# Giuseppe5/brevitas

Measured on AMD Instinct MI355X. Metric: Gelem/s fused int8 fake-quant fwd+bwd, per-channel, [256,512,56,56], higher is better.
Workload: dtype bf16

## Files before the change

### brevitas_amd/_native.py

```python
import ctypes
import os

import torch

_PKG = os.path.dirname(os.path.abspath(__file__))
LIB_PATH = os.environ.get('BREVITAS_AMD_LIB') or os.path.join(_PKG, 'libbvq.so')

F32, BF16, F16 = 0, 1, 2
ROUND, FLOOR, CEIL, ROUND_TO_ZERO, DPU_ROUND = range(5)
(OP_ROUND, OP_FLOOR, OP_CEIL, OP_ROUND_TO_ZERO, OP_DPU_ROUND, OP_BINARY_SIGN, OP_TERNARY_SIGN,
 OP_ABS) = range(8)
STAT_ABSMAX, STAT_MINMAX = 0, 1
SCALAR_OPMATH, SCALAR_CAST = 0, 1
OUT_DEQUANT, OUT_INT = 0, 1
MATCH_ABS, MATCH_VALUE = 0, 1
MATCH_FIRST = 16
PRE_NONE, PRE_RELU = 0, 1
CODES_I32, CODES_I8, CODES_U8 = 0, 1, 2
_CODES_TORCH = {CODES_I32: torch.int32, CODES_I8: torch.int8, CODES_U8: torch.uint8}
ABI_VERSION = 2

_DTYPES = {torch.float32: F32, torch.bfloat16: BF16, torch.float16: F16}

EXPORTS = (
    'bvq_abi_version', 'bvq_last_error', 'bvq_unary', 'bvq_stats_pre', 'bvq_scalar_clamp', 'bvq_tensor_clamp',
    'bvq_tensor_clamp_bwd', 'bvq_abs_binary_sign_grad_bwd', 'bvq_stats_workspace_bytes', 'bvq_stats',
    'bvq_absmax_scale', 'bvq_running_stats_update', 'bvq_scale_from_stat', 'bvq_shard_pack', 'bvq_shard_unpack', 'bvq_abs_moments_workspace_bytes', 'bvq_abs_moments',
    'bvq_abs_affine_bwd', 'bvq_kth_workspace_bytes', 'bvq_kth_value', 'bvq_kth_pair', 'bvq_kth_passes',
    'bvq_kth_hist_offset', 'bvq_kth_begin', 'bvq_kth_hist', 'bvq_kth_pick', 'bvq_kth_finish', 'bvq_stat_bwd', 'bvq_tie_info_bytes', 'bvq_stat_tie_scan', 'bvq_stat_tie_apply', 'bvq_stat_tie_apply_dscale', 'bvq_fakequant_fwd', 'bvq_stats_fakequant_fwd_workspace_bytes', 'bvq_stats_fakequant_fwd',
    'bvq_fakequant_bwd_workspace_bytes', 'bvq_fakequant_bwd_stats_workspace_bytes', 'bvq_fakequant_bwd_stats', 'bvq_fakequant_bwd',
    'bvq_learned_scale', 'bvq_fakequant_bwd_learned', 'bvq_variant_fwd', 'bvq_variant_bwd_workspace_bytes', 'bvq_variant_bwd',
    'bvq_fakequant_fwd_bounds', 'bvq_fakequant_bwd_bounds', 'bvq_histc', 'bvq_absmax_scale_running', 'bvq_selftest_div_f16r',
    'bvq_kthw_plan', 'bvq_kthw_begin', 'bvq_kthw_hist', 'bvq_kthw_pick', 'bvq_kthw_finish',
    'bvq_absmax_onepass_supported', 'bvq_absmax_scale_onepass', 'bvq_fakequant_bwd_stats_onepass_supported',
    'bvq_fakequant_bwd_stats_onepass', 'bvq_scale_from_stat_running', 'bvq_fakequant_bwd_shard',
    'bvq_shard_unpack_deposit', 'bvq_absmax_list_supported', 'bvq_absmax_scale_list', 'bvq_weight_list_supported',
    'bvq_weight_quant_list_fwd', 'bvq_weight_quant_list_bwd_workspace_bytes', 'bvq_weight_quant_list_bwd')


class QuantDesc(ctypes.Structure):
    _fields_ = [
        ('outer', ctypes.c_int64), ('channels', ctypes.c_int64), ('inner', ctypes.c_int64),
        ('x_dtype', ctypes.c_int32), ('ct_dtype', ctypes.c_int32), ('scale_dtype', ctypes.c_int32),
        ('zp_dtype', ctypes.c_int32), ('scale_per_channel', ctypes.c_int32),
        ('zp_per_channel', ctypes.c_int32), ('qmin', ctypes.c_float), ('qmax', ctypes.c_float),
        ('round_mode', ctypes.c_int32), ('scalar_mode', ctypes.c_int32), ('clamp_ste', ctypes.c_int32),
        ('out_kind', ctypes.c_int32), ('pre_op', ctypes.c_int32), ('codes_dtype', ctypes.c_int32)]


class VariantDesc(ctypes.Structure):
    _fields_ = [
        ('outer', ctypes.c_int64), ('channels', ctypes.c_int64), ('inner', ctypes.c_int64), ('kind', ctypes.c_int32),
        ('x_dtype', ctypes.c_int32), ('ct_dtype', ctypes.c_int32), ('scale_dtype', ctypes.c_int32),
        ('zp_dtype', ctypes.c_int32), ('scale_per_channel', ctypes.c_int32), ('round_mode', ctypes.c_int32),
        ('clamp_ste', ctypes.c_int32), ('scalar_mode', ctypes.c_int32), ('qmin', ctypes.c_float),
        ('qmax', ctypes.c_float), ('threshold', ctypes.c_float), ('trunc_scale', ctypes.c_float)]


VAR_BINARY, VAR_CLAMPED_BINARY, VAR_TERNARY, VAR_DECOUPLED, VAR_TRUNC = range(5)

WEIGHT_LIST_MAX = 16


class WeightItem(ctypes.Structure):
    _fields_ = [
        ('x', ctypes.c_void_p), ('y', ctypes.c_void_p), ('stat', ctypes.c_void_p), ('scale', ctypes.c_void_p),
        ('g', ctypes.c_void_p), ('dx', ctypes.c_void_p), ('dscale', ctypes.c_void_p), ('channels', ctypes.c_int64),
        ('inner', ctypes.c_int64), ('min_val', ctypes.c_double), ('int_threshold', ctypes.c_double),
        ('qmin', ctypes.c_float), ('qmax', ctypes.c_float), ('use_min', ctypes.c_int32), ('clamp_ste', ctypes.c_int32)]


class BvqError(RuntimeError):
    pass


def _load(path=None, strict=True):
    path = path or LIB_PATH
    if not os.path.exists(path):
        raise ImportError(
            'brevitas_amd: %s is missing. Build it with `python -m brevitas_amd.csrc.build` '
            '(needs hipcc, gfx950). There is no fallback backend.' % path)
    lib = ctypes.CDLL(path)
    vp, i64, i32, dbl = ctypes.c_void_p, ctypes.c_int64, ctypes.c_int, ctypes.c_double
    lib.bvq_abi_version.restype = i32
    lib.bvq_last_error.restype = ctypes.c_char_p
    sig = {
        'bvq_unary': (i32, [i32, i32, vp, vp, i64, vp]),
        'bvq_scalar_clamp': (i32, [i32, vp, vp, i64, dbl, i32, dbl, i32, vp]),
        'bvq_tensor_clamp': (i32, [i32, vp, vp, vp, i32, vp, i64, vp]),
        'bvq_tensor_clamp_bwd': (i32, [i32, vp, vp, vp, vp, i32, vp, i64, vp]),
        'bvq_abs_binary_sign_grad_bwd': (i32, [i32, vp, vp, vp, i64, vp]),
        'bvq_stats_workspace_bytes': (i64, [i32, i32, i64, i64, i64]),
        'bvq_stats': (i32, [i32, i32, vp, i64, i64, i64, i32, vp, vp, i64, vp]),
        'bvq_stats_pre': (i32, [i32, i32, i32, vp, i64, i64, i64, i32, vp, vp, i64, vp]),
        'bvq_stat_bwd': (i32, [i32, i32, vp, vp, vp, vp, i64, i64, i64, i32, vp, i64, vp]),
        'bvq_fakequant_fwd': (i32, [ctypes.POINTER(QuantDesc), vp, vp, vp, vp, vp, vp]),
        'bvq_stats_fakequant_fwd_workspace_bytes': (i64, [ctypes.POINTER(QuantDesc), vp, vp]),
        'bvq_stats_fakequant_fwd': (i32, [ctypes.POINTER(QuantDesc), vp, dbl, i32, dbl, vp, vp, vp, vp, i64, vp]),
        'bvq_fakequant_bwd_workspace_bytes': (i64, [ctypes.POINTER(QuantDesc)]),
        'bvq_fakequant_bwd_stats_workspace_bytes': (i64, [ctypes.POINTER(QuantDesc)]),
        'bvq_fakequant_bwd_stats': (i32, [ctypes.POINTER(QuantDesc), vp, vp, vp, vp, vp, vp, vp, i32, dbl, i32, vp, i64, vp]),
        'bvq_fakequant_bwd_stats_onepass_supported': (i32, [ctypes.POINTER(QuantDesc)]),
        'bvq_fakequant_bwd_stats_onepass': (i32, [ctypes.POINTER(QuantDesc), vp, vp, vp, vp, vp, vp, vp, i32, dbl, i32, vp, i64, vp, i64, vp]),
        'bvq_absmax_scale': (i32, [i32, i32, vp, i64, i64, i64, vp, dbl, i32, dbl, i32, vp, vp, i64, vp]),
        'bvq_absmax_scale_running': (i32, [i32, i32, vp, i64, i64, i64, vp, dbl, i32, dbl, i32, vp, i32, vp, dbl, i32, vp, i64, vp]),
        'bvq_absmax_onepass_supported': (i32, [i32, vp, i64, i64, i64]),
        'bvq_absmax_scale_onepass': (i32, [i32, i32, vp, i64, i64, i64, i32, vp, dbl, i32, dbl, i32, vp, i32, vp, dbl, i32, vp, i64, vp]),
        'bvq_absmax_list_supported': (i32, [i32, i32, vp, vp, i64, vp]),
        'bvq_absmax_scale_list': (i32, [i32, i32, vp, vp, i64, vp, vp, dbl, i32, dbl, i32, vp, vp, i64, vp, i64, vp]),
        'bvq_running_stats_update': (i32, [i32, vp, i32, vp, i64, dbl, i32, vp]),
        'bvq_scale_from_stat': (i32, [vp, i64, i32, vp, dbl, i32, dbl, i32, vp, vp]),
        'bvq_scale_from_stat_running': (i32, [vp, i64, i32, vp, dbl, i32, dbl, i32, vp, i32, vp, dbl, i32, vp]),
        'bvq_fakequant_bwd_shard': (i32, [ctypes.POINTER(QuantDesc), vp, vp, vp, vp, vp, vp, vp, vp, i32, vp, i64, vp, i64, vp]),
        'bvq_shard_unpack_deposit': (i32, [i32, vp, vp, vp, i32, i64, i32, vp, i64, i32, dbl, i32, i32, vp, vp]),
        'bvq_shard_pack': (i32, [vp, vp, i64, i32, i32, vp, vp]),
        'bvq_shard_unpack': (i32, [vp, i32, i64, i32, i32, vp, vp, vp, vp]),
        'bvq_abs_moments_workspace_bytes': (i64, [i32, i64, i64, i64]),
        'bvq_abs_moments': (i32, [i32, vp, i64, i64, i64, vp, vp, i64, vp]),
        'bvq_abs_affine_bwd': (i32, [i32, vp, vp, vp, vp, i64, i64, i64, vp]),
        'bvq_kth_workspace_bytes': (i64, [i32, i64, i64, i64]),
        'bvq_kth_value': (i32, [i32, i32, vp, i64, i64, i64, i64, vp, vp, i64, vp]),
        'bvq_kth_pair': (i32, [i32, i32, vp, i64, i64, i64, i64, i64, vp, vp, i64, vp]),
        'bvq_kth_passes': (i32, [i32]),
        'bvq_kth_hist_offset': (i64, [i32, i64, i32]),
        'bvq_kth_begin': (i32, [i32, i64, i32, i64, dbl, vp, i64, vp]),
        'bvq_kth_hist': (i32, [i32, i32, vp, i64, i64, i64, i32, vp, i64, vp]),
        'bvq_kth_pick': (i32, [i32, i64, i32, i32, dbl, vp, i64, vp]),
        'bvq_kth_finish': (i32, [i32, i32, i64, vp, vp, i64, vp]),
        'bvq_kthw_plan': (i32, [i32, i32, i32, vp, vp]),
        'bvq_kthw_begin': (i32, [i32, i32, vp, i64, vp]),
        'bvq_kthw_hist': (i32, [i32, i32, vp, i64, i32, vp, i64, vp]),
        'bvq_kthw_pick': (i32, [i32, i32, i32, i32, i64, dbl, vp, i64, vp]),
        'bvq_kthw_finish': (i32, [i32, i32, vp, vp, i64, vp]),
        'bvq_tie_info_bytes': (i64, [i64]),
        'bvq_stat_tie_scan': (i32, [i32, i32, vp, vp, i64, i64, i64, vp, vp, vp]),
        'bvq_stat_tie_apply': (i32, [i32, i32, i32, vp, vp, vp, vp, vp, vp, i64, i64, i64, i32, vp]),
        'bvq_stat_tie_apply_dscale': (i32, [i32, i32, vp, vp, vp, i32, dbl, i32, vp, vp, vp, i64, i64, i64, vp]),
        'bvq_fakequant_bwd': (i32, [ctypes.POINTER(QuantDesc), vp, vp, vp, vp, vp, vp, vp, vp, vp, vp, i64, vp]),
        'bvq_learned_scale': (i32, [i32, vp, i64, dbl, i32, dbl, i32, vp, vp]),
        'bvq_histc': (i32, [i32, vp, i64, vp, i32, vp, vp]),
        'bvq_selftest_div_f16r': (i32, [vp, i32, vp, i32, vp, vp]),
        'bvq_fakequant_fwd_bounds': (i32, [ctypes.POINTER(QuantDesc), vp, vp, vp, vp, vp, vp]),
        'bvq_fakequant_bwd_bounds': (i32, [ctypes.POINTER(QuantDesc), vp, vp, vp, vp, vp, vp, vp, vp, vp, i64, vp]),
        'bvq_variant_fwd': (i32, [ctypes.POINTER(VariantDesc), vp, vp, vp, vp, vp, vp, vp]),
        'bvq_variant_bwd_workspace_bytes': (i64, [ctypes.POINTER(VariantDesc)]),
        'bvq_variant_bwd': (i32, [ctypes.POINTER(VariantDesc), vp, vp, vp, vp, vp, vp, vp, vp, vp, vp, i64, vp]),
        'bvq_weight_list_supported': (i32, [i32, i32, i32, vp, i64]),
        'bvq_weight_quant_list_fwd': (i32, [i32, i32, i32, i32, vp, vp]),
        'bvq_weight_quant_list_bwd_workspace_bytes': (i64, [i32, i32, vp]),
        'bvq_weight_quant_list_bwd': (i32, [i32, i32, i32, i32, i32, vp, vp, i64, vp, i64, vp]),
        'bvq_fakequant_bwd_learned': (i32, [ctypes.POINTER(QuantDesc), vp, vp, vp, vp, vp, vp, vp, i32, dbl, i32, dbl, vp, vp, vp, i64, vp]),
    }
    for name, (res, args) in sig.items():
        fn = getattr(lib, name, None)
        if fn is None:
            if strict:
                raise ImportError('brevitas_amd: %s does not export %s' % (path, name))
            continue
        fn.restype = res
        fn.argtypes = args
    ver = lib.bvq_abi_version()
    if ver != ABI_VERSION:
        raise ImportError('brevitas_amd: libbvq.so has ABI %d, this package needs %d' % (ver, ABI_VERSION))
    return lib


lib = _load()


def last_error():
    return lib.bvq_last_error().decode()


def check(rc, what):
    if rc != 0:
        raise BvqError('%s failed (%d): %s' % (what, rc, last_error()))


def dtype_code(dtype):
    try:
        return _DTYPES[dtype]
    except KeyError:
        raise BvqError('brevitas_amd: unsupported dtype %s (float32, bfloat16, float16)' % dtype)


def require_device(*tensors):
    dev = None
    for t in tensors:
        if t is None:
            continue
        if not t.is_cuda:
            raise BvqError(
                'brevitas_amd: got a %s tensor; the fake-quantization engine only runs on a ROCm '
                'device (there is no CPU fallback)' % t.device)
        if dev is None:
            dev = t.device
        elif t.device != dev:
            raise BvqError('brevitas_amd: tensors on different devices (%s, %s)' % (dev, t.device))
    return dev


_raw_stream = getattr(torch._C, '_cuda_getCurrentRawStream', None)


def stream_ptr(device):
    if _raw_stream is not None:
        return _raw_stream(device.index if device.index is not None else torch.cuda.current_device())
    return torch.cuda.current_stream(device).cuda_stream


def ptr(t):
    return t.data_ptr() if t is not None else None


class _DeviceGuard:
    __slots__ = ('ctx',)

    def __init__(self, dev):
        idx = dev.index
        self.ctx = None if idx is None or idx == torch.cuda.current_device() else torch.cuda.device(dev)

    def __enter__(self):
        if self.ctx is not None:
            self.ctx.__enter__()

    def __exit__(self, *exc):
        if self.ctx is not None:
            self.ctx.__exit__(*exc)
        return False


_timer = None


def set_kernel_timer(timer):
    global _timer
    _timer = timer


ARRIVE_WORDS = 1 << 16
_arrive = {}
ONEPASS = True
ONEPASS_BWD = True


def arrival_buffer(dev, stream, words):
    if not ONEPASS or words > ARRIVE_WORDS:
        return None
    key = (dev.index, stream)
    buf = _arrive.get(key)
    if buf is None:
        if torch.cuda.is_current_stream_capturing():
            return None
        buf = _arrive[key] = torch.zeros(ARRIVE_WORDS, dtype=torch.int32, device=dev)
    return buf



def unary(op, x):
    dev = require_device(x)
    x = x.contiguous()
    y = torch.empty_like(x)
    with _DeviceGuard(dev):
        check(lib.bvq_unary(op, dtype_code(x.dtype), ptr(x), ptr(y), x.numel(), stream_ptr(dev)), 'bvq_unary')
    return y


def scalar_clamp(x, lo, hi):
    dev = require_device(x)
    x = x.contiguous()
    y = torch.empty_like(x)
    with _DeviceGuard(dev):
        check(lib.bvq_scalar_clamp(dtype_code(x.dtype), ptr(x), ptr(y), x.numel(),
                                   0.0 if lo is None else float(lo), int(lo is not None),
                                   0.0 if hi is None else float(hi), int(hi is not None), stream_ptr(dev)),
              'bvq_scalar_clamp')
    return y


def _bounds(x, lo, hi):
    lo = lo.to(device=x.device, dtype=x.dtype)
    hi = hi.to(device=x.device, dtype=x.dtype)
    if lo.numel() == 1 and hi.numel() == 1:
        return lo.reshape(1), hi.reshape(1), 0
    return lo.expand_as(x).contiguous(), hi.expand_as(x).contiguous(), 1


def tensor_clamp(x, lo, hi, out=None):
    dev = require_device(x)
    xc = x.contiguous()
    lo, hi, full = _bounds(xc, lo, hi)
    y = out if out is not None else torch.empty_like(xc)
    with _DeviceGuard(dev):
        check(lib.bvq_tensor_clamp(dtype_code(xc.dtype), ptr(xc), ptr(lo), ptr(hi), full, ptr(y), xc.numel(),
                                   stream_ptr(dev)), 'bvq_tensor_clamp')
    return y


def tensor_clamp_bwd(g, x, lo, hi):
    dev = require_device(g, x)
    xc = x.contiguous()
    g = g.to(xc.dtype).contiguous()
    lo, hi, full = _bounds(xc, lo, hi)
    dx = torch.empty_like(xc)
    with _DeviceGuard(dev):
        check(lib.bvq_tensor_clamp_bwd(dtype_code(xc.dtype), ptr(g), ptr(xc), ptr(lo), ptr(hi), full, ptr(dx),
                                       xc.numel(), stream_ptr(dev)), 'bvq_tensor_clamp_bwd')
    return dx


def abs_binary_sign_grad_bwd(g, x):
    dev = require_device(g, x)
    xc = x.contiguous()
    g = g.to(xc.dtype).contiguous()
    dx = torch.empty_like(xc)
    with _DeviceGuard(dev):
        check(lib.bvq_abs_binary_sign_grad_bwd(dtype_code(xc.dtype), ptr(g), ptr(xc), ptr(dx), xc.numel(),
                                               stream_ptr(dev)), 'bvq_abs_binary_sign_grad_bwd')
    return dx


def stats(kind, x, outer, channels, inner, out_f32=False, pre_op=PRE_NONE):
    dev = require_device(x)
    assert x.is_contiguous() and x.numel() == outer * channels * inner
    dt = dtype_code(x.dtype)
    nout = channels * (2 if kind == STAT_MINMAX else 1)
    out = torch.empty(nout, dtype=torch.float32 if out_f32 else x.dtype, device=dev)
    if kind == STAT_ABSMAX and lib.bvq_absmax_onepass_supported(dt, ptr(x), outer, channels, inner):
        with _DeviceGuard(dev):
            st = stream_ptr(dev)
            arrive = arrival_buffer(dev, st, max(2 * channels, 18))
            if arrive is not None:
                if _timer is not None:
                    _timer.before('bvq_stats')
                check(lib.bvq_absmax_scale_onepass(pre_op, dt, ptr(x), outer, channels, inner, dtype_code(out.dtype),
                                                   ptr(out), 0.0, 0, 1.0, 0, None, 0, None, 0.0, 0, ptr(arrive),
                                                   arrive.numel(), st), 'bvq_absmax_scale_onepass')
                if _timer is not None:
                    _timer.after('bvq_stats')
                return out
    wsb = lib.bvq_stats_workspace_bytes(kind, dt, outer, channels, inner)
    if wsb < 0:
        raise BvqError('bvq_stats_workspace_bytes: bad arguments')
    ws = torch.empty(max(int(wsb), 8), dtype=torch.uint8, device=dev)
    with _DeviceGuard(dev):
        if _timer is not None:
            _timer.before('bvq_stats')
        check(lib.bvq_stats_pre(kind, pre_op, dt, ptr(x), outer, channels, inner, dtype_code(out.dtype), ptr(out),
                                ptr(ws), ws.numel(), stream_ptr(dev)), 'bvq_stats')
        if _timer is not None:
            _timer.after('bvq_stats')
    return out


def stat_bwd(match, x, stat, gstat, outer, channels, inner, dx=None):
    dev = require_device(x, stat, gstat, dx)
    assert x.is_contiguous()
    dt = dtype_code(x.dtype)
    stat = stat.to(x.dtype).contiguous()
    gstat = gstat.to(x.dtype).contiguous()
    mode_add = int(dx is not None)
    if dx is None:
        dx = torch.empty_like(x)
    assert dx.is_contiguous() and dx.dtype == x.dtype
    wsb = lib.bvq_stats_workspace_bytes(STAT_ABSMAX, dt, outer, channels, inner)
    ws = torch.empty(max(int(wsb), 8), dtype=torch.uint8, device=dev)
    with _DeviceGuard(dev):
        check(lib.bvq_stat_bwd(match, dt, ptr(x), ptr(stat), ptr(gstat), ptr(dx), outer, channels, inner,
                               mode_add, ptr(ws), ws.numel(), stream_ptr(dev)), 'bvq_stat_bwd')
    return dx


def fakequant_fwd(desc, x, scale, zp, want_codes=False, want_y=True):
    dev = require_device(x, scale, zp)
    ct = {F32: torch.float32, BF16: torch.bfloat16, F16: torch.float16}[desc.ct_dtype]
    y = torch.empty(x.shape, dtype=ct, device=dev) if want_y else None
    codes = torch.empty(x.shape, dtype=_CODES_TORCH[desc.codes_dtype], device=dev) if want_codes else None
    with _DeviceGuard(dev):
        if _timer is not None:
            _timer.before('bvq_fakequant_fwd')
        check(lib.bvq_fakequant_fwd(ctypes.byref(desc), ptr(x), ptr(scale), ptr(zp), ptr(y), ptr(codes),
                                    stream_ptr(dev)), 'bvq_fakequant_fwd')
        if _timer is not None:
            _timer.after('bvq_fakequant_fwd')
    if not want_y:
        return codes
    return (y, codes) if want_codes else y


def stats_fakequant_fwd(desc, x, min_val, int_threshold, scale_dtype):
    dev = require_device(x)
    assert x.is_contiguous()
    y = torch.empty_like(x)
    wsb = int(lib.bvq_stats_fakequant_fwd_workspace_bytes(ctypes.byref(desc), ptr(x), ptr(y)))
    if wsb <= 0:
        return None
    channels = int(desc.channels) if (desc.scale_per_channel and desc.channels > 1) else 1
    stat = torch.empty(channels, dtype=x.dtype, device=dev)
    scale = torch.empty(channels, dtype=scale_dtype, device=dev)
    ws = torch.empty(wsb, dtype=torch.uint8, device=dev)
    with _DeviceGuard(dev):
        if _timer is not None:
            _timer.before('bvq_stats_fakequant_fwd')
        check(lib.bvq_stats_fakequant_fwd(ctypes.byref(desc), ptr(x), float(min_val or 0.0), int(bool(min_val)),
                                          float(int_threshold), ptr(stat), ptr(scale), ptr(y), ptr(ws), wsb,
                                          stream_ptr(dev)), 'bvq_stats_fakequant_fwd')
        if _timer is not None:
            _timer.after('bvq_stats_fakequant_fwd')
    return stat, scale, y


def absmax_scale_list(xs, outers, channels, inners, min_val, int_threshold, scale_dtype):
    dev = require_device(*xs)
    n = len(xs)
    dt = dtype_code(xs[0].dtype)
    for x, o, i in zip(xs, outers, inners):
        assert x.is_contiguous() and x.dtype == xs[0].dtype and x.numel() == o * channels * i
    ptrs = (ctypes.c_void_p * n)(*[x.data_ptr() for x in xs])
    oa = (ctypes.c_int64 * n)(*outers)
    ia = (ctypes.c_int64 * n)(*inners)
    if not lib.bvq_absmax_list_supported(dt, n, ptrs, oa, channels, ia):
        return None
    with _DeviceGuard(dev):
        st = stream_ptr(dev)
        arrive = ws = None
        if channels > 1:
            arrive = arrival_buffer(dev, st, max(2 * channels, 18))
            if arrive is None:
                return None
        else:
            ws = torch.empty(1 << 14, dtype=torch.uint8, device=dev)
        stat = torch.empty(channels, dtype=xs[0].dtype, device=dev)
        scale = torch.empty(channels, dtype=scale_dtype, device=dev)
        check(lib.bvq_absmax_scale_list(dt, n, ptrs, oa, channels, ia, ptr(stat), float(min_val or 0.0),
                                        int(bool(min_val)), float(int_threshold), dtype_code(scale_dtype), ptr(scale),
                                        ptr(arrive), arrive.numel() if arrive is not None else 0, ptr(ws),
                                        ws.numel() if ws is not None else 0, st), 'bvq_absmax_scale_list')
    return stat, scale


def absmax_scale(x, outer, channels, inner, min_val, int_threshold, scale_dtype, pre_op=PRE_NONE, running=None,
                 momentum=0.0, first_batch=False):
    dev = require_device(x)
    assert x.is_contiguous() and x.numel() == outer * channels * inner
    dt = dtype_code(x.dtype)
    stat = torch.empty(channels, dtype=x.dtype, device=dev)
    scale = torch.empty(channels, dtype=scale_dtype, device=dev)
    if lib.bvq_absmax_onepass_supported(dt, ptr(x), outer, channels, inner):
        with _DeviceGuard(dev):
            st = stream_ptr(dev)
            arrive = arrival_buffer(dev, st, max(2 * channels, 18))
            if arrive is not None:
                if _timer is not None:
                    _timer.before('bvq_stats')
                check(lib.bvq_absmax_scale_onepass(
                    pre_op, dt, ptr(x), outer, channels, inner, dt, ptr(stat), float(min_val or 0.0),
                    int(bool(min_val)), float(int_threshold), dtype_code(scale_dtype), ptr(scale),
                    dtype_code(running.dtype) if running is not None else 0, ptr(running), float(momentum),
                    int(first_batch), ptr(arrive), arrive.numel(), st), 'bvq_absmax_scale_onepass')
                if _timer is not None:
                    _timer.after('bvq_stats')
                return stat, scale
    wsb = lib.bvq_stats_workspace_bytes(STAT_ABSMAX, dt, outer, channels, inner)
    ws = torch.empty(max(int(wsb), 8), dtype=torch.uint8, device=dev)
    with _DeviceGuard(dev):
        if _timer is not None:
            _timer.before('bvq_stats')
        if running is not None:
            check(lib.bvq_absmax_scale_running(pre_op, dt, ptr(x), outer, channels, inner, ptr(stat),
                                               float(min_val or 0.0), int(bool(min_val)), float(int_threshold),
                                               dtype_code(scale_dtype), ptr(scale), dtype_code(running.dtype),
                                               ptr(running), float(momentum), int(first_batch), ptr(ws), ws.numel(),
                                               stream_ptr(dev)), 'bvq_absmax_scale_running')
        else:
            check(lib.bvq_absmax_scale(pre_op, dt, ptr(x), outer, channels, inner, ptr(stat), float(min_val or 0.0),
                                       int(bool(min_val)), float(int_threshold), dtype_code(scale_dtype), ptr(scale),
                                       ptr(ws), ws.numel(), stream_ptr(dev)), 'bvq_absmax_scale')
        if _timer is not None:
            _timer.after('bvq_stats')
    return stat, scale


def kth_value(x, k, outer, channels, inner, abs_key):
    dev = require_device(x)
    assert x.is_contiguous() and x.numel() == outer * channels * inner
    dt = dtype_code(x.dtype)
    out = torch.empty(channels, dtype=x.dtype, device=dev)
    wsb = int(lib.bvq_kth_workspace_bytes(dt, outer, channels, inner))
    if wsb < 0:
        raise BvqError('bvq_kth_workspace_bytes: bad arguments')
    ws = torch.empty(wsb, dtype=torch.uint8, device=dev)
    with _DeviceGuard(dev):
        if _timer is not None:
            _timer.before('bvq_kth_value')
        check(lib.bvq_kth_value(int(abs_key), dt, ptr(x), outer, channels, inner, int(k), ptr(out), ptr(ws), wsb,
                                stream_ptr(dev)), 'bvq_kth_value')
        if _timer is not None:
            _timer.after('bvq_kth_value')
    return out


def kth_pair(x, k_first, k_second, outer, channels, inner, abs_key):
    dev = require_device(x)
    assert x.is_contiguous() and x.numel() == outer * channels * inner
    dt = dtype_code(x.dtype)
    out = torch.empty(2, channels, dtype=x.dtype, device=dev)
    wsb = int(lib.bvq_kth_workspace_bytes(dt, outer, channels, inner))
    if wsb < 0:
        raise BvqError('bvq_kth_workspace_bytes: bad arguments')
    ws = torch.empty(wsb, dtype=torch.uint8, device=dev)
    with _DeviceGuard(dev):
        check(lib.bvq_kth_pair(int(abs_key), dt, ptr(x), outer, channels, inner, int(k_first), int(k_second), ptr(out),
                               ptr(ws), wsb, stream_ptr(dev)), 'bvq_kth_pair')
    return out


KTH_EXPLICIT, KTH_HIGH, KTH_LOW = 0, 1, 2
_KBINS = 2048


def scale_from_stat(stat32, stat_dtype, min_val, int_threshold, scale_dtype, running=None, momentum=0.0,
                    first_batch=False):
    dev = require_device(stat32, running)
    assert stat32.dtype == torch.float32 and stat32.is_contiguous()
    n = stat32.numel()
    stat = torch.empty(n, dtype=stat_dtype, device=dev)
    scale = torch.empty(n, dtype=scale_dtype, device=dev)
    with _DeviceGuard(dev):
        check(lib.bvq_scale_from_stat_running(
            ptr(stat32), n, dtype_code(stat_dtype), ptr(stat), float(min_val or 0.0), int(bool(min_val)),
            float(int_threshold), dtype_code(scale_dtype), ptr(scale),
            dtype_code(running.dtype) if running is not None else 0, ptr(running), float(momentum), int(first_batch),
            stream_ptr(dev)), 'bvq_scale_from_stat_running')
    return stat, scale


def fakequant_bwd_shard(desc, g, x, scale, zp, stat, rank):
    dev = require_device(g, x, scale, zp, stat)
    wsb = int(lib.bvq_fakequant_bwd_stats_workspace_bytes(ctypes.byref(desc)))
    if wsb <= 0 or (x.data_ptr() | g.data_ptr()) & 15:
        return None
    ch = int(desc.channels)
    dx = torch.empty_like(x)
    msg = torch.empty(2 * ch, dtype=torch.float64, device=dev)
    pos = torch.empty(ch, dtype=torch.int64, device=dev)
    ws = torch.empty(wsb, dtype=torch.uint8, device=dev)
    stat = stat.to(x.dtype).contiguous()
    with _DeviceGuard(dev):
        st = stream_ptr(dev)
        arrive = arrival_buffer(dev, st, ch) if ONEPASS_BWD else None
        if _timer is not None:
            _timer.before('bvq_fakequant_bwd')
        check(lib.bvq_fakequant_bwd_shard(ctypes.byref(desc), ptr(g), ptr(x), ptr(scale), ptr(zp), ptr(stat), ptr(dx),
                                          ptr(msg), ptr(pos), int(rank), ptr(ws), wsb, ptr(arrive),
                                          arrive.numel() if arrive is not None else 0, st), 'bvq_fakequant_bwd_shard')
        if _timer is not None:
            _timer.after('bvq_fakequant_bwd')
    return dx, msg, pos

# ... 447 lines not shown
```

### brevitas_amd/core/quant/_fused.py

```python
from typing import NamedTuple, Optional

import torch
from torch import Tensor
from torch.autograd import Function

import brevitas_amd.config as config
from brevitas_amd import _native as nat

_FLOATS = (torch.float32, torch.bfloat16, torch.float16)


class Plan(NamedTuple):
    outer: int
    channels: int
    inner: int
    scale_pc: bool
    zp_pc: bool
    ct: torch.dtype
    nhwc: bool = False


def is_nhwc(x: Tensor, channel_dim) -> bool:
    return channel_dim == 1 and x.dim() == 4 and not x.is_contiguous() \
        and x.is_contiguous(memory_format=torch.channels_last)
# ... 182 lines not shown
        gy = _like_memory_order(gy.to(ct), ctx.back)
        gs = gscale.reshape(-1).contiguous().to(sc.dtype) if gscale is not None else None
        dx, _, dvalue = nat.fakequant_bwd_learned(desc, gy, xc, sc, zp.reshape(-1), value, min_val, thr_div, gs)
        if not ctx.needs_input_grad[0]:
            dx = None
        elif ctx.back is not None:
            dx = dx.permute(ctx.back)
        return dx, dvalue.view(value.shape), None, None, None, None, None, None, None, None, None


class VariantFn(Function):

    @staticmethod
    def forward(ctx, x, scale, pre_scale, zp, pre_zp, p, opts):
        xc = x.contiguous()
        sc = scale.reshape(-1).contiguous()
        ps = pre_scale.reshape(-1).contiguous() if pre_scale is not None else None
        zc = zp.reshape(-1).contiguous() if zp is not None else None
        pz = pre_zp.reshape(-1).contiguous() if pre_zp is not None else None
        zdt = (zc if zc is not None else pz if pz is not None else _zero_zero_point(x.device)).dtype
        desc = nat.VariantDesc(p.outer, p.channels, p.inner, opts['kind'], nat.dtype_code(x.dtype),
                               nat.dtype_code(opts['ct']), nat.dtype_code(sc.dtype), nat.dtype_code(zdt), int(p.scale_pc),
                               opts.get('round_mode', nat.ROUND), int(opts.get('clamp_ste', False)), scalar_mode(),
                               opts.get('qmin', 0.0), opts.get('qmax', 0.0), opts.get('threshold', 0.0),
                               opts.get('trunc_scale', 1.0))
        y = nat.variant_fwd(desc, xc, sc, ps, zc, pz)
        ctx.desc = desc
        ctx.save_for_backward(xc, sc, ps, zc, pz)
        ctx.shapes = (scale.shape, scale.dtype, None if pre_scale is None else (pre_scale.shape, pre_scale.dtype))
        return y

    @staticmethod
    def backward(ctx, gy):
        xc, sc, ps, zc, pz = ctx.saved_tensors
        desc = ctx.desc
        ct = {nat.F32: torch.float32, nat.BF16: torch.bfloat16, nat.F16: torch.float16}[desc.ct_dtype]
        need_ds, need_dp = ctx.needs_input_grad[1], ctx.needs_input_grad[2] and ps is not None
        dx, ds, dp = nat.variant_bwd(desc, gy.to(ct).contiguous(), xc, sc, ps, zc, pz, need_ds, need_dp)
        sshape, sdt, pre = ctx.shapes
        ds = ds.reshape(sshape).to(sdt) if need_ds else None
        dp = dp.reshape(pre[0]).to(pre[1]) if need_dp else None
        return (dx if ctx.needs_input_grad[0] else None), ds, dp, None, None, None, None


def _dimensioned_wider_scalar(x: Tensor, t: Optional[Tensor]) -> bool:
    return t is not None and t.numel() == 1 and t.dim() > 0 and torch.promote_types(x.dtype, t.dtype) != x.dtype


def variant_plan(x: Tensor, scale: Tensor, *others: Optional[Tensor]) -> Optional[Plan]:
    if not config.FUSED_PATHS or torch._C._get_tracing_state() is not None:
        return None
    if _dimensioned_wider_scalar(x, scale):
        return None
    p = plan(x, scale, _zero_zero_point(x.device) if x.is_cuda else scale)
    if p is None or p.nhwc or not x.is_contiguous():
        return None
    for t in others:
        if t is not None and (t.shape != scale.shape or t.dtype != scale.dtype or not t.is_cuda):
            return None
    return p


def scalar_zero_point_ok(*zps: Optional[Tensor], x: Optional[Tensor] = None) -> bool:
    return all(z is None or (z.numel() == 1 and z.is_cuda and z.dtype in _FLOATS and not z.requires_grad
                             and not (x is not None and _dimensioned_wider_scalar(x, z))) for z in zps)


class StatsPlan(NamedTuple):
    outer: int
    channels: int
    inner: int
    scaling_shape: tuple
    min_val: float
    int_threshold: float
    nhwc: bool = False


_ZERO_ZP = {}


def _zero_zero_point(device):
    z = _ZERO_ZP.get(device)
    if z is None:
        z = torch.zeros((), dtype=torch.float32, device=device)
        _ZERO_ZP[device] = z
    return z


_AS_DTYPE = {}


def _as_dtype_value(v: float, dtype: torch.dtype) -> float:
    key = (v, dtype)
    r = _AS_DTYPE.get(key)
    if r is None:
        r = _AS_DTYPE[key] = float(torch.tensor(v, dtype=torch.float32).to(dtype))
    return r


def stats_scale(flat: Tensor, int_threshold: Tensor, sp, group, pre_op, running=None):
    if group is None:
        if len(sp.scaling_shape) > 0:
            scale_dtype, thr_div = flat.dtype, _as_dtype_value(sp.int_threshold, flat.dtype)
        else:
            scale_dtype = torch.promote_types(flat.dtype, int_threshold.dtype)
            thr_div = sp.int_threshold
        if running is not None:
            buf, momentum, first = running
            stat, scale = nat.absmax_scale(flat, sp.outer, sp.channels, sp.inner, sp.min_val, thr_div, scale_dtype,
                                           pre_op, running=buf, momentum=momentum, first_batch=first)
        else:
            stat, scale = nat.absmax_scale(flat, sp.outer, sp.channels, sp.inner, sp.min_val, thr_div, scale_dtype,
                                           pre_op)
        return stat, scale.view(sp.scaling_shape)
    from brevitas_amd.distributed import sync_stat_max
    stat32 = sync_stat_max(nat.stats(nat.STAT_ABSMAX, flat, sp.outer, sp.channels, sp.inner, out_f32=True,
                                     pre_op=pre_op), group)
    if len(sp.scaling_shape) > 0:
        scale_dtype, thr_div = flat.dtype, _as_dtype_value(sp.int_threshold, flat.dtype)
    else:
        scale_dtype = torch.promote_types(flat.dtype, int_threshold.dtype)
        thr_div = sp.int_threshold
    if running is not None:
        buf, momentum, first = running
        stat, scale = nat.scale_from_stat(stat32, flat.dtype, sp.min_val, thr_div, scale_dtype, buf, momentum, first)
    else:
        stat, scale = nat.scale_from_stat(stat32, flat.dtype, sp.min_val, thr_div, scale_dtype)
    return stat, scale.view(sp.scaling_shape)


class StatsFakeQuantFn(Function):

    @staticmethod
    def forward(ctx, x, int_threshold, sp, qmin, qmax, round_mode, clamp_ste, group=None, pre_op=nat.PRE_NONE,
                runtime=None):
        ctx.set_materialize_grads(False)
        ctx.pre_op = pre_op
        xc, back = _memory_order(x, sp.channels, sp.nhwc)
        ctx.back = back
        flat = xc.reshape(-1)
        zp = _zero_zero_point(x.device)
        fused = None
        if group is None and config.FUSED_PATHS and x.dtype in _FLOATS:
            if len(sp.scaling_shape) > 0:
                scale_dtype, thr_div = x.dtype, _as_dtype_value(sp.int_threshold, x.dtype)
            else:
                scale_dtype = torch.promote_types(x.dtype, int_threshold.dtype)
                thr_div = sp.int_threshold
            code = nat.dtype_code(x.dtype)
            desc = nat.QuantDesc(sp.outer, sp.channels, sp.inner, code, code, nat.dtype_code(scale_dtype),
                                 nat.dtype_code(zp.dtype), int(sp.channels > 1), 0, qmin, qmax, round_mode,
                                 scalar_mode(), int(clamp_ste), nat.OUT_DEQUANT, pre_op)
            fused = nat.stats_fakequant_fwd(desc, xc, sp.min_val, thr_div, scale_dtype)
        if fused is not None:
            stat, scale, y = fused
            scale = scale.view(sp.scaling_shape)
        else:
            running = None
            if runtime is not None:
                buf = runtime.running_stats
                if buf.is_cuda and buf.is_contiguous() and buf.numel() == sp.channels and buf.dtype in _FLOATS:
                    running = (buf, runtime.momentum, runtime.first_batch)
                    runtime.bvq_running_folded = True
            stat, scale = stats_scale(flat, int_threshold, sp, group, pre_op, running)
            p = Plan(sp.outer, sp.channels, sp.inner, sp.channels > 1, False, torch.result_type(x, scale), sp.nhwc)
            if not (p.ct == x.dtype or p.ct == torch.float32):
                raise nat.BvqError('StatsFakeQuantFn: unsupported operand layout (caller must pre-check)')
            sc = scale.reshape(-1).contiguous()
            desc = make_desc(p, xc, sc, zp.reshape(-1), qmin, qmax, round_mode, clamp_ste, nat.OUT_DEQUANT, pre_op)
            y = nat.fakequant_fwd(desc, xc, sc, zp.reshape(-1))
        ctx.desc = desc
        ctx.sp = sp
        ctx.group = group
        ctx.save_for_backward(xc, scale, zp, stat, int_threshold)
        stat_out = stat.view(sp.scaling_shape)
        ctx.mark_non_differentiable(stat_out)
        if back is not None:
            y = y.permute(back)
        return y, scale, stat_out

    @staticmethod
    def backward(ctx, gy, gscale, _gstat):
        xc, scale, zp, stat, int_threshold = ctx.saved_tensors
        dx = stats_backward(xc, scale, zp, stat, int_threshold, ctx.desc, ctx.sp, ctx.group, ctx.pre_op, ctx.back, gy,
                            gscale)
        return dx, None, None, None, None, None, None, None, None, None


class StatsGraphFakeQuantFn(Function):

    @staticmethod
    def forward(ctx, x, int_threshold, sp, qmin, qmax, round_mode, clamp_ste, pre_op, post, *params):
        ctx.set_materialize_grads(False)
        xc, back = _memory_order(x, sp.channels, sp.nhwc)
        flat = xc.reshape(-1)
        stat = nat.stats(nat.STAT_ABSMAX, flat, sp.outer, sp.channels, sp.inner, pre_op=pre_op).view(sp.scaling_shape)
        with torch.enable_grad():
            s_leaf = stat.detach().requires_grad_(True)
            scale_g = post(s_leaf) / int_threshold
        scale = scale_g.detach()
        zp = _zero_zero_point(x.device)
        p = plan(xc if back is None else x, scale, zp)
        if p is None or p.zp_pc or p.nhwc != sp.nhwc:
            raise nat.BvqError('StatsGraphFakeQuantFn: operand layout not covered by the quantizer kernels')
        sc = scale.reshape(-1).contiguous()
        desc = make_desc(p, xc, sc, zp.reshape(-1), qmin, qmax, round_mode, clamp_ste, nat.OUT_DEQUANT, pre_op)
        y = nat.fakequant_fwd(desc, xc, sc, zp.reshape(-1))
        ctx.desc, ctx.sp, ctx.back, ctx.pre_op = desc, sp, back, pre_op
        ctx.graph = (s_leaf, scale_g, params)
        ctx.save_for_backward(xc, scale, zp, stat)
        ctx.mark_non_differentiable(stat)
        if back is not None:
            y = y.permute(back)
        return y, scale, stat

    @staticmethod
    def backward(ctx, gy, gscale, _gstat):
        xc, scale, zp, stat = ctx.saved_tensors
        desc, sp = ctx.desc, ctx.sp
        s_leaf, scale_g, params = ctx.graph
        none = (None,) * 9
        ct = {nat.F32: torch.float32, nat.BF16: torch.bfloat16, nat.F16: torch.float16}[desc.ct_dtype]
        if gy is None and gscale is None:
            return none + (None,) * len(params)
        if gy is None:
            gy = torch.zeros(xc.shape, dtype=ct, device=xc.device)
        else:
            gy = _like_memory_order(gy.to(ct), ctx.back)
        stat_x = stat.reshape(-1).to(xc.dtype).contiguous()
        dx, ds, _, ties = nat.fakequant_bwd(desc, gy, xc, scale.reshape(-1).contiguous(), zp.reshape(-1), True, False,
                                            tie_stat=stat_x)
        dscale = _reduce_like(ds, scale)
        if gscale is not None:
            dscale = dscale + gscale
        grads = torch.autograd.grad(scale_g, (s_leaf,) + tuple(params), dscale, retain_graph=True, allow_unused=True)
        dstat = grads[0]
        if dstat is not None:
            nat.stat_tie_apply(nat.MATCH_ABS, xc.reshape(-1), stat_x, dstat.reshape(-1).to(xc.dtype).contiguous(), ties,
                               dx.reshape(-1), sp.outer, sp.channels, sp.inner, mode_add=True, pre_op=ctx.pre_op)
        return (_restore(dx, ctx.back),) + none[1:] + tuple(grads[1:])


def _list_views(params, sp):
    flats = [t.detach().reshape(-1) for t in params]
    return flats, [1] * len(params), [t.numel() // sp.channels for t in params]


def list_stats_supported(params, sp) -> bool:
    import ctypes
    if not config.FUSED_PATHS or params[0].dtype not in _FLOATS or sp.outer != 1 or sp.nhwc:
        return False
    flats, outers, inners = _list_views(params, sp)
    n = len(flats)
    st = nat.stream_ptr(flats[0].device)
    if sp.channels > 1 and nat.arrival_buffer(flats[0].device, st, max(2 * sp.channels, 18)) is None:
        return False
    return bool(nat.lib.bvq_absmax_list_supported(
        nat.dtype_code(flats[0].dtype), n, (ctypes.c_void_p * n)(*[f.data_ptr() for f in flats]),
        (ctypes.c_int64 * n)(*outers), sp.channels, (ctypes.c_int64 * n)(*inners)))


class ListStatsFakeQuantFn(Function):

    @staticmethod
    def forward(ctx, x, int_threshold, sp, qmin, qmax, round_mode, clamp_ste, index, *params):
        ctx.set_materialize_grads(False)
        flats, outers, inners = _list_views(params, sp)
        if len(sp.scaling_shape) > 0:
            scale_dtype, thr_div = x.dtype, _as_dtype_value(sp.int_threshold, x.dtype)
        else:
            scale_dtype = torch.promote_types(x.dtype, int_threshold.dtype)
            thr_div = sp.int_threshold
        out = nat.absmax_scale_list(flats, outers, sp.channels, inners, sp.min_val, thr_div, scale_dtype)
        if out is None:
            raise nat.BvqError('ListStatsFakeQuantFn: list not covered (caller must pre-check list_stats_supported)')
        stat, scale = out
        scale = scale.view(sp.scaling_shape)
        zp = _zero_zero_point(x.device)
        xc = x.detach()
        p = Plan(sp.outer, sp.channels, sp.inner, sp.channels > 1, False, torch.result_type(x, scale), False)
        if not (p.ct == x.dtype or p.ct == torch.float32):
            raise nat.BvqError('ListStatsFakeQuantFn: unsupported operand layout')
        sc = scale.reshape(-1).contiguous()
        desc = make_desc(p, xc, sc, zp.reshape(-1), qmin, qmax, round_mode, clamp_ste, nat.OUT_DEQUANT, nat.PRE_NONE)
        y = nat.fakequant_fwd(desc, xc, sc, zp.reshape(-1))
        ctx.desc, ctx.sp, ctx.index, ctx.inners = desc, sp, index, inners
        ctx.save_for_backward(scale, zp, stat, int_threshold, *params)
        stat_out = stat.view(sp.scaling_shape)
        ctx.mark_non_differentiable(stat_out)
        return y, scale, stat_out

    @staticmethod
    def backward(ctx, gy, gscale, _gstat):
        scale, zp, stat, int_threshold = ctx.saved_tensors[:4]
        params = ctx.saved_tensors[4:]
        desc, sp, index = ctx.desc, ctx.sp, ctx.index
        none = (None,) * 8
        if gy is None and gscale is None:
            return none + (None,) * len(params)
        x = params[index].detach()
        ct = {nat.F32: torch.float32, nat.BF16: torch.bfloat16, nat.F16: torch.float16}[desc.ct_dtype]
        gy = torch.zeros(x.shape, dtype=ct, device=x.device) if gy is None else gy.to(ct).contiguous()
        stat_x = stat.reshape(-1).to(x.dtype).contiguous()
        dx, ds, _, own = nat.fakequant_bwd(desc, gy, x, scale.reshape(-1).contiguous(), zp.reshape(-1), True, False,
                                           tie_stat=stat_x)
        ds = _reduce_like(ds, scale)
# ... 261 lines not shown
```

### brevitas_amd/csrc/build.py

```python
import hashlib
import os
import shutil
import subprocess
import sys
from concurrent.futures import ThreadPoolExecutor

CSRC = os.path.dirname(os.path.abspath(__file__))
PKG = os.path.dirname(CSRC)
ROOT = os.path.dirname(PKG)
LIB = os.path.join(PKG, 'libbvq.so')
OBJ_DIR = os.path.join(ROOT, 'build', 'bvq')

SOURCES = [('bvq_common.hip', [], 'bvq_common.o'), ('bvq_elementwise.hip', [], 'bvq_elementwise.o'),
           ('bvq_stats.hip', [], 'bvq_stats.o'), ('bvq_select.hip', [], 'bvq_select.o'),
           ('bvq_variants.hip', [], 'bvq_variants.o'), ('bvq_fakequant_fwd.hip', [], 'bvq_fakequant_fwd.o'),
           ('bvq_fakequant_bwd.hip', [], 'bvq_fakequant_bwd.o'),
           ('bvq_fakequant_bwd_bf16.hip', [], 'bvq_fakequant_bwd_bf16.o'),
           ('bvq_fakequant_bwd_f16.hip', [], 'bvq_fakequant_bwd_f16.o'),
           ('bvq_fakequant_bwd_f32.hip', [], 'bvq_fakequant_bwd_f32.o'),
           ('bvq_weight_list.hip', [], 'bvq_weight_list.o')]
HEADERS = ['bvq_common.h', 'bvq_quant_math.h', 'bvq_ties.h', 'bvq_sums.h', 'bvq_fakequant.h', 'bvq_fakequant_bwd.h',
           os.path.join(ROOT, 'include', 'bvq.h')]

FLAGS = [
    '--offload-arch=gfx950', '-O3', '-std=c++17', '-fPIC', '-ffp-contract=off', '-fno-fast-math', '--offload-compress',
    '-Wall', '-Wno-unused-function', '-Wno-sometimes-uninitialized', '-Wno-uninitialized',
    '-Wno-unused-variable']


def _hipcc():
    for cand in (os.environ.get('HIPCC'), shutil.which('hipcc'), '/opt/rocm/bin/hipcc'):
        if cand and os.path.exists(cand):
            return cand
    raise RuntimeError('hipcc not found: brevitas_amd needs the ROCm toolchain to build libbvq.so')


def _digest():
    h = hashlib.sha256()
    for f in sorted(set(src for src, _, _ in SOURCES)) + HEADERS + [os.path.abspath(__file__)]:
        path = f if os.path.isabs(f) else os.path.join(CSRC, f)
        with open(path, 'rb') as fh:
            h.update(fh.read())
    h.update(' '.join(FLAGS).encode())
    return h.hexdigest()


def source_digest():
    stamp = os.path.join(OBJ_DIR, 'stamp')
    dig = _digest()
    if os.path.exists(LIB) and os.path.exists(stamp):
        with open(stamp) as fh:
            if fh.read().strip() == dig:
                return dig
    return None


def build(force=False, verbose=False, defines=(), out=None):
    lib_path = out or LIB
    obj_dir = OBJ_DIR if not out else os.path.join(OBJ_DIR, os.path.basename(out).replace('.', '_'))
    stamp = os.path.join(obj_dir, 'stamp')
    dig = (_digest() + ' ' + ' '.join(defines)).strip()
    if not force and os.path.exists(lib_path) and os.path.exists(stamp):
        with open(stamp) as fh:
            if fh.read().strip() == dig:
                return lib_path
    os.makedirs(obj_dir, exist_ok=True)
    hipcc = _hipcc()

    def compile_one(item):
        src, part_defines, objname = item
        obj = os.path.join(obj_dir, objname)
        cmd = [hipcc] + FLAGS + ['-D' + d for d in list(defines) + part_defines] + \
            ['-c', os.path.join(CSRC, src), '-o', obj]
        if verbose:
            print(' '.join(cmd), flush=True)
        r = subprocess.run(cmd, capture_output=True, text=True)
        if r.returncode != 0:
            raise RuntimeError('hipcc failed on %s:\n%s\n%s' % (src, r.stdout, r.stderr))
        if verbose and r.stderr.strip():
            print(r.stderr, flush=True)
        return obj

    with ThreadPoolExecutor(max_workers=8) as ex:
        objs = list(ex.map(compile_one, SOURCES))
    cmd = [hipcc, '--offload-arch=gfx950', '-shared', '-fPIC', '-o', lib_path + '.tmp'] + objs
    r = subprocess.run(cmd, capture_output=True, text=True)
    if r.returncode != 0:
        raise RuntimeError('link failed:\n%s\n%s' % (r.stdout, r.stderr))
    os.replace(lib_path + '.tmp', lib_path)
    with open(stamp, 'w') as fh:
        fh.write(dig)
    return lib_path


AUTOGRAD_SO = os.path.join(PKG, '_bvq_autograd.so')


def build_autograd(force=False, verbose=False):
    src = os.path.join(CSRC, 'bvq_autograd.cpp')
    import torch
    h = hashlib.sha256()
    for path in (src, os.path.join(ROOT, 'include', 'bvq.h')):
        with open(path, 'rb') as fh:
            h.update(fh.read())
    h.update(torch.__version__.encode())
    stamp = os.path.join(ROOT, 'build', 'autograd', 'stamp')
    if not force and os.path.exists(AUTOGRAD_SO) and os.path.exists(stamp):
        with open(stamp) as fh:
            if fh.read().strip() == h.hexdigest():
                return AUTOGRAD_SO
    from torch.utils import cpp_extension
    bdir = os.path.join(ROOT, 'build', 'autograd')
    os.makedirs(bdir, exist_ok=True)
    cpp_extension.load(name='_bvq_autograd', sources=[src], build_directory=bdir, extra_cflags=['-O2', '-std=c++17', '-D__HIP_PLATFORM_AMD__=1'],
                       extra_include_paths=[os.path.join(ROOT, 'include'), os.path.join(os.environ.get('ROCM_PATH', '/opt/rocm'), 'include')],
                       extra_ldflags=['-ldl'], verbose=verbose, is_python_module=False)
    built = os.path.join(bdir, '_bvq_autograd.so')
    shutil.copyfile(built, AUTOGRAD_SO)
    with open(stamp, 'w') as fh:
        fh.write(h.hexdigest())
    return AUTOGRAD_SO


if __name__ == '__main__':
    defs = [a[2:] for a in sys.argv[1:] if a.startswith('-D')]
    outs = [a.split('=', 1)[1] for a in sys.argv[1:] if a.startswith('--out=')]
    print(build(force='--force' in sys.argv, verbose='-v' in sys.argv, defines=defs,
                out=os.path.abspath(outs[0]) if outs else None))
```

### brevitas_amd/csrc/bvq_autograd.cpp

```cpp
#include <dlfcn.h>
#include <rccl/rccl.h>
#include <torch/csrc/distributed/c10d/ProcessGroup.hpp>
#include <torch/extension.h>

#include <cstdint>
#include <cstring>
#include <stdexcept>
#include <string>
#include <unordered_map>

#include "bvq.h"

namespace {

#define BVQ_ENTRIES(X)                       \
  X(bvq_abi_version)                         \
  X(bvq_last_error)                          \
  X(bvq_stats_fakequant_fwd_workspace_bytes) \
  X(bvq_stats_fakequant_fwd)                 \
  X(bvq_fakequant_bwd_stats_workspace_bytes) \
  X(bvq_fakequant_bwd_stats)                 \
  X(bvq_fakequant_bwd_stats_onepass_supported) \
  X(bvq_fakequant_bwd_stats_onepass)         \
  X(bvq_absmax_onepass_supported)            \
  X(bvq_absmax_scale_onepass)                \
  X(bvq_stats_workspace_bytes)               \
  X(bvq_stats_pre)                           \
  X(bvq_absmax_scale)                        \
  X(bvq_absmax_scale_running)                \
  X(bvq_scale_from_stat_running)             \
  X(bvq_fakequant_fwd)                       \
  X(bvq_fakequant_bwd_workspace_bytes)       \
  X(bvq_fakequant_bwd)                       \
  X(bvq_tie_info_bytes)                      \
  X(bvq_stat_tie_apply_dscale)               \
  X(bvq_fakequant_bwd_shard)                 \
  X(bvq_shard_unpack_deposit)                \
  X(bvq_shard_pack)                          \
  X(bvq_shard_unpack)
#define BVQ_DECLARE(name) decltype(&name) p_##name = nullptr;
BVQ_ENTRIES(BVQ_DECLARE)
#undef BVQ_DECLARE

py::object* g_fallback = nullptr;

void check(int rc, const char* what) {
  if (rc != 0) throw std::runtime_error(std::string(what) + ": " + (p_bvq_last_error ? p_bvq_last_error() : "error"));
}

at::ScalarType dtype_of(int code) {
  return code == BVQ_F32 ? at::kFloat : (code == BVQ_BF16 ? at::kBFloat16 : at::kHalf);
}
int code_of(at::ScalarType t) { return t == at::kFloat ? BVQ_F32 : (t == at::kBFloat16 ? BVQ_BF16 : BVQ_F16); }

bool aligned16(const at::Tensor& t) { return (reinterpret_cast<uintptr_t>(t.data_ptr()) & 15) == 0; }

struct Params {
  bvq_quant_desc d;
  double min_val, thr_fwd, thr_bwd, thr_raw;
  int has_min, scale_dtype;
  int64_t stream;
  std::vector<int64_t> shape;
  int quot_dtype = BVQ_F32;
  double momentum = 0.0;
  int first_batch = 0;
  c10::intrusive_ptr<c10d::ProcessGroup> group;
  py::object py_group;
};

struct GroupRef {
  c10::intrusive_ptr<c10d::ProcessGroup> pg;
  py::object* py;
};
std::unordered_map<std::string, GroupRef>& groups() {
  static auto* m = new std::unordered_map<std::string, GroupRef>();
  return *m;
}

struct Rccl {
  decltype(&ncclGetUniqueId) get_unique_id = nullptr;
  decltype(&ncclCommInitRank) comm_init_rank = nullptr;
  decltype(&ncclCommDestroy) comm_destroy = nullptr;
  decltype(&ncclAllReduce) all_reduce = nullptr;
  decltype(&ncclAllGather) all_gather = nullptr;
  decltype(&ncclGetErrorString) error_string = nullptr;
  bool ok = false;
};
const Rccl& rccl() {
  static const Rccl r = [] {
    Rccl t;
    void* h = nullptr;
    for (const char* name : {"librccl.so", "librccl.so.1"}) {
      h = dlopen(name, RTLD_NOW | RTLD_NOLOAD);
      if (h) break;
    }
    if (!h) return t;
    t.get_unique_id = reinterpret_cast<decltype(t.get_unique_id)>(dlsym(h, "ncclGetUniqueId"));
    t.comm_init_rank = reinterpret_cast<decltype(t.comm_init_rank)>(dlsym(h, "ncclCommInitRank"));
    t.comm_destroy = reinterpret_cast<decltype(t.comm_destroy)>(dlsym(h, "ncclCommDestroy"));
    t.all_reduce = reinterpret_cast<decltype(t.all_reduce)>(dlsym(h, "ncclAllReduce"));
    t.all_gather = reinterpret_cast<decltype(t.all_gather)>(dlsym(h, "ncclAllGather"));
    t.error_string = reinterpret_cast<decltype(t.error_string)>(dlsym(h, "ncclGetErrorString"));
    t.ok = t.get_unique_id && t.comm_init_rank && t.comm_destroy && t.all_reduce && t.all_gather && t.error_string;
    return t;
  }();
  return r;
}
void rccl_check(ncclResult_t rc, const char* what) {
  if (rc != ncclSuccess) throw std::runtime_error(std::string(what) + ": " + rccl().error_string(rc));
}
struct NativeComm {
  ncclComm_t comm;
  int world, rank;
};
std::unordered_map<std::string, NativeComm>& native_comms() {
  static auto* m = new std::unordered_map<std::string, NativeComm>();
  return *m;
}
const NativeComm* native_comm(const std::string& name) {
  auto it = native_comms().find(name);
  return it == native_comms().end() ? nullptr : &it->second;
}

std::vector<int64_t> desc_ints(const Params& p) {
  return {p.d.outer, p.d.channels, p.d.inner, p.d.x_dtype, p.d.ct_dtype, p.d.scale_dtype, p.d.zp_dtype,
          p.d.scale_per_channel, p.d.zp_per_channel, p.d.round_mode, p.d.scalar_mode, p.d.clamp_ste, p.d.out_kind,
          p.d.pre_op, p.d.codes_dtype, p.scale_dtype, p.stream, p.quot_dtype};
}
bvq_quant_desc desc_from(const std::vector<int64_t>& dv, const std::vector<double>& qr) {
  bvq_quant_desc d;
  d.outer = dv[0];
  d.channels = dv[1];
  d.inner = dv[2];
  d.x_dtype = (int32_t)dv[3];
  d.ct_dtype = (int32_t)dv[4];
  d.scale_dtype = (int32_t)dv[5];
  d.zp_dtype = (int32_t)dv[6];
  d.scale_per_channel = (int32_t)dv[7];
  d.zp_per_channel = (int32_t)dv[8];
  d.qmin = (float)qr[0];
  d.qmax = (float)qr[1];
  d.round_mode = (int32_t)dv[9];
  d.scalar_mode = (int32_t)dv[10];
  d.clamp_ste = (int32_t)dv[11];
  d.out_kind = (int32_t)dv[12];
  d.pre_op = (int32_t)dv[13];
  d.codes_dtype = (int32_t)dv[14];
  return d;
}

bool direct_gradient(const at::Tensor& gy, const at::Tensor& gscale, const at::Tensor& x) {
  return gy.defined() && !gscale.defined() && gy.is_contiguous() && gy.scalar_type() == x.scalar_type() && aligned16(gy) &&
         aligned16(x);
}

torch::autograd::variable_list python_backward(torch::autograd::AutogradContext* ctx, const at::Tensor& gy,
                                               const at::Tensor& gscale, const py::object* group, size_t n_inputs) {
  const auto saved = ctx->get_saved_variables();
  torch::autograd::variable_list out(n_inputs);
  if (!gy.defined() && !gscale.defined()) return out;
  py::gil_scoped_acquire gil;
  py::object dx = (*g_fallback)(saved[0], saved[1], saved[2], saved[3], saved[4],
                                py::cast(ctx->saved_data["desc"].toIntVector()),
                                py::cast(ctx->saved_data["qrange"].toDoubleVector()),
                                py::cast(ctx->saved_data["shape"].toIntVector()), gy.defined() ? py::cast(gy) : py::none(),
                                gscale.defined() ? py::cast(gscale) : py::none(), group ? *group : py::none());
  out[0] = dx.cast<at::Tensor>();
  return out;
}

class StatsFakeQuant : public torch::autograd::Function<StatsFakeQuant> {
 public:
  static torch::autograd::variable_list forward(torch::autograd::AutogradContext* ctx, const at::Tensor& x,
                                                const at::Tensor& zp, const at::Tensor& int_threshold,
                                                const at::Tensor& arrive, int64_t wsb, const Params& p) {
    ctx->set_materialize_grads(false);
    const int64_t ch = p.d.channels;
    at::Tensor y = at::empty_like(x);
    at::Tensor stat = at::empty({ch}, x.options());
    at::Tensor scale = at::empty({ch}, x.options().dtype(dtype_of(p.scale_dtype)));
    at::Tensor ws = at::empty({wsb}, x.options().dtype(at::kByte));
    check(p_bvq_stats_fakequant_fwd(&p.d, x.data_ptr(), p.min_val, p.has_min, p.thr_fwd, stat.data_ptr(),
                                    scale.data_ptr(), y.data_ptr(), ws.data_ptr(), wsb,
                                    reinterpret_cast<void*>(p.stream)),
          "bvq_stats_fakequant_fwd");
    ctx->save_for_backward({x, scale, zp, stat, int_threshold, arrive});
    ctx->saved_data["desc"] = desc_ints(p);
    ctx->saved_data["qrange"] = std::vector<double>{p.d.qmin, p.d.qmax, p.thr_bwd, p.thr_raw};
    ctx->saved_data["shape"] = p.shape;
    at::Tensor scale_out = scale.view(p.shape), stat_out = stat.view(p.shape);
    ctx->mark_non_differentiable({stat_out});
    return {y, scale_out, stat_out};
  }

  static torch::autograd::variable_list backward(torch::autograd::AutogradContext* ctx,
                                                 torch::autograd::variable_list grads) {
    const auto saved = ctx->get_saved_variables();
    const at::Tensor &x = saved[0], &scale = saved[1], &zp = saved[2], &stat = saved[3], &arrive = saved[5];
    const at::Tensor& gy = grads[0];
    const at::Tensor& gscale = grads[1];
    if (!direct_gradient(gy, gscale, x)) return python_backward(ctx, gy, gscale, nullptr, 6);
    const auto dv = ctx->saved_data["desc"].toIntVector();
    const auto qr = ctx->saved_data["qrange"].toDoubleVector();
    const bvq_quant_desc d = desc_from(dv, qr);
    const int64_t wsb = p_bvq_fakequant_bwd_stats_workspace_bytes(&d);
    if (wsb <= 0) throw std::runtime_error("bvq_fakequant_bwd_stats: layout not covered (checked at forward)");
    at::Tensor dx = at::empty_like(x);
    at::Tensor ds = at::empty({d.channels}, x.options().dtype(at::kFloat));
    at::Tensor ws = at::empty({wsb}, x.options().dtype(at::kByte));
    const int sdt = (int)dv[15];
    void* st = reinterpret_cast<void*>(dv[16]);
    if (arrive.numel() >= d.channels && p_bvq_fakequant_bwd_stats_onepass_supported(&d)) {
      check(p_bvq_fakequant_bwd_stats_onepass(&d, gy.data_ptr(), x.data_ptr(), scale.data_ptr(), zp.data_ptr(),
                                              stat.data_ptr(), dx.data_ptr(), ds.data_ptr<float>(), sdt, qr[2], sdt,
                                              ws.data_ptr(), wsb, reinterpret_cast<uint32_t*>(arrive.data_ptr()),
                                              arrive.numel(), st),
            "bvq_fakequant_bwd_stats_onepass");
    } else {
      check(p_bvq_fakequant_bwd_stats(&d, gy.data_ptr(), x.data_ptr(), scale.data_ptr(), zp.data_ptr(), stat.data_ptr(),
                                      dx.data_ptr(), ds.data_ptr<float>(), sdt, qr[2], sdt, ws.data_ptr(), wsb, st),
            "bvq_fakequant_bwd_stats");
    }
    torch::autograd::variable_list out(6);
    out[0] = dx;
    return out;
  }
};

class ActStatsFakeQuant : public torch::autograd::Function<ActStatsFakeQuant> {
 public:
  static torch::autograd::variable_list forward(torch::autograd::AutogradContext* ctx, const at::Tensor& x,
                                                const at::Tensor& zp, const at::Tensor& int_threshold,
                                                const at::Tensor& running, const at::Tensor& arrive, const Params& p) {
    ctx->set_materialize_grads(false);
    const bvq_quant_desc& d = p.d;
    const int64_t ch = d.channels;
    void* st = reinterpret_cast<void*>(p.stream);
    const bool sharded = (bool)p.group;
    const auto xdt = x.scalar_type();
    at::Tensor stat = at::empty({ch}, x.options());
    at::Tensor scale = at::empty({ch}, x.options().dtype(dtype_of(p.scale_dtype)));
    at::Tensor stat32;
    if (sharded) stat32 = at::empty({ch}, x.options().dtype(at::kFloat));
    const bool has_running = running.numel() > 0, has_arrive = arrive.numel() > 0;
    void* run_ptr = has_running ? running.data_ptr() : nullptr;
    const int run_dt = has_running ? code_of(running.scalar_type()) : BVQ_F32;
    const bool onepass = has_arrive &&
                         p_bvq_absmax_onepass_supported(d.x_dtype, x.data_ptr(), d.outer, ch, d.inner);
    if (onepass) {
      check(p_bvq_absmax_scale_onepass(d.pre_op, d.x_dtype, x.data_ptr(), d.outer, ch, d.inner,
                                       sharded ? BVQ_F32 : d.x_dtype, sharded ? stat32.data_ptr() : stat.data_ptr(),
                                       p.min_val, p.has_min, p.thr_fwd, p.scale_dtype,
                                       sharded ? nullptr : scale.data_ptr(), run_dt, sharded ? nullptr : run_ptr, p.momentum,
                                       p.first_batch, reinterpret_cast<uint32_t*>(arrive.data_ptr()), arrive.numel(), st),
            "bvq_absmax_scale_onepass");
    } else {
      const int64_t wsb = p_bvq_stats_workspace_bytes(BVQ_STAT_ABSMAX, d.x_dtype, d.outer, ch, d.inner);
      if (wsb < 0) throw std::runtime_error("bvq_stats_workspace_bytes: bad arguments");
      at::Tensor ws = at::empty({wsb > 8 ? wsb : 8}, x.options().dtype(at::kByte));
      if (sharded) {
        check(p_bvq_stats_pre(BVQ_STAT_ABSMAX, d.pre_op, d.x_dtype, x.data_ptr(), d.outer, ch, d.inner, BVQ_F32,
                              stat32.data_ptr(), ws.data_ptr(), ws.numel(), st),
              "bvq_stats_pre");
      } else if (has_running) {
        check(p_bvq_absmax_scale_running(d.pre_op, d.x_dtype, x.data_ptr(), d.outer, ch, d.inner, stat.data_ptr(),
                                         p.min_val, p.has_min, p.thr_fwd, p.scale_dtype, scale.data_ptr(), run_dt, run_ptr,
                                         p.momentum, p.first_batch, ws.data_ptr(), ws.numel(), st),
              "bvq_absmax_scale_running");
      } else {
        check(p_bvq_absmax_scale(d.pre_op, d.x_dtype, x.data_ptr(), d.outer, ch, d.inner, stat.data_ptr(), p.min_val,
                                 p.has_min, p.thr_fwd, p.scale_dtype, scale.data_ptr(), ws.data_ptr(), ws.numel(), st),
              "bvq_absmax_scale");
      }
    }
    if (sharded) {
      if (const NativeComm* nc = native_comm(p.group->getGroupName())) {
        rccl_check(rccl().all_reduce(stat32.data_ptr<float>(), stat32.data_ptr<float>(), (size_t)ch, ncclFloat32, ncclMax,
                                     nc->comm, reinterpret_cast<hipStream_t>(st)),
                   "ncclAllReduce");
      } else {
        std::vector<at::Tensor> ts{stat32};
        c10d::AllreduceOptions opts;
        opts.reduceOp = c10d::ReduceOp::MAX;
        p.group->allreduce(ts, opts)->wait();
      }
      check(p_bvq_scale_from_stat_running(stat32.data_ptr<float>(), ch, d.x_dtype, stat.data_ptr(), p.min_val, p.has_min,
                                          p.thr_fwd, p.scale_dtype, scale.data_ptr(), run_dt, run_ptr, p.momentum,
                                          p.first_batch, st),
            "bvq_scale_from_stat_running");
    }
    at::Tensor y = at::empty(x.sizes(), x.options().dtype(dtype_of(d.ct_dtype)));
    check(p_bvq_fakequant_fwd(&d, x.data_ptr(), scale.data_ptr(), zp.data_ptr(), y.data_ptr(), nullptr, st),
          "bvq_fakequant_fwd");
    ctx->save_for_backward({x, scale, zp, stat, int_threshold, arrive});
    ctx->saved_data["desc"] = desc_ints(p);
    ctx->saved_data["qrange"] = std::vector<double>{d.qmin, d.qmax, p.thr_bwd, p.thr_raw};
    ctx->saved_data["shape"] = p.shape;
    if (sharded) {
      const std::string name = p.group->getGroupName();
      auto it = groups().find(name);
      if (it == groups().end()) {
        groups()[name] = GroupRef{p.group, new py::object(p.py_group)};
      } else if (it->second.pg != p.group) {
        it->second.pg = p.group;
        *it->second.py = p.py_group;
      }
      ctx->saved_data["group"] = name;
    }
    at::Tensor scale_out = scale.view(p.shape), stat_out = stat.view(p.shape);
    ctx->mark_non_differentiable({stat_out});
    return {y, scale_out, stat_out};
  }

  static torch::autograd::variable_list backward(torch::autograd::AutogradContext* ctx,
                                                 torch::autograd::variable_list grads) {
    const auto saved = ctx->get_saved_variables();
    const at::Tensor &x = saved[0], &scale = saved[1], &zp = saved[2], &stat = saved[3], &arrive = saved[5];
    const at::Tensor& gy = grads[0];
    const at::Tensor& gscale = grads[1];
    const auto dv = ctx->saved_data["desc"].toIntVector();
    const auto qr = ctx->saved_data["qrange"].toDoubleVector();
    const bvq_quant_desc d = desc_from(dv, qr);
    c10::intrusive_ptr<c10d::ProcessGroup> group;
    py::object* py_group = nullptr;
    if (ctx->saved_data.count("group")) {
      const GroupRef& ref = groups().at(ctx->saved_data["group"].toStringRef());
      group = ref.pg;
      py_group = ref.py;
    }
    const bool per_channel = d.channels > 1;
    if (!direct_gradient(gy, gscale, x)) {
      return python_backward(ctx, gy, gscale, py_group, 6);
    }
    void* st = reinterpret_cast<void*>(dv[16]);
    const int sdt = (int)dv[15];
    at::Tensor dx = at::empty_like(x);
    torch::autograd::variable_list out(6);
    if (per_channel) {
      const int64_t wsb = p_bvq_fakequant_bwd_stats_workspace_bytes(&d);
      if (wsb <= 0) throw std::runtime_error("bvq_fakequant_bwd_stats: layout not covered (checked at forward)");
      at::Tensor ws = at::empty({wsb}, x.options().dtype(at::kByte));
      uint32_t* arr = arrive.numel() > 0 ? reinterpret_cast<uint32_t*>(arrive.data_ptr()) : nullptr;
      const int64_t arr_n = arrive.numel();
      if (group) {
        const int rank = group->getRank(), world = group->getSize();
        at::Tensor msg = at::empty({2 * d.channels}, x.options().dtype(at::kDouble));
        at::Tensor pos = at::empty({d.channels}, x.options().dtype(at::kLong));
        check(p_bvq_fakequant_bwd_shard(&d, gy.data_ptr(), x.data_ptr(), scale.data_ptr(), zp.data_ptr(), stat.data_ptr(),
                                        dx.data_ptr(), msg.data_ptr<double>(), pos.data_ptr<int64_t>(), rank, ws.data_ptr(),
                                        wsb, arr, arr_n, st),
              "bvq_fakequant_bwd_shard");
        at::Tensor gathered = at::empty({world * msg.numel()}, msg.options());
        if (const NativeComm* nc = native_comm(group->getGroupName())) {
          rccl_check(rccl().all_gather(msg.data_ptr<double>(), gathered.data_ptr<double>(), (size_t)msg.numel(),
                                       ncclFloat64, nc->comm, reinterpret_cast<hipStream_t>(st)),
                     "ncclAllGather");
        } else {
          group->_allgather_base(gathered, msg)->wait();
        }
        check(p_bvq_shard_unpack_deposit(d.x_dtype, x.data_ptr(), dx.data_ptr(), gathered.data_ptr<double>(), world,
                                         d.channels, rank, pos.data_ptr<int64_t>(), d.inner, sdt, qr[2], sdt, d.pre_op,
                                         nullptr, st),
              "bvq_shard_unpack_deposit");
      } else {
        at::Tensor ds = at::empty({d.channels}, x.options().dtype(at::kFloat));
        if (arr && arr_n >= d.channels && p_bvq_fakequant_bwd_stats_onepass_supported(&d)) {
          check(p_bvq_fakequant_bwd_stats_onepass(&d, gy.data_ptr(), x.data_ptr(), scale.data_ptr(), zp.data_ptr(),
                                                  stat.data_ptr(), dx.data_ptr(), ds.data_ptr<float>(), sdt, qr[2], sdt,
                                                  ws.data_ptr(), wsb, arr, arr_n, st),
                "bvq_fakequant_bwd_stats_onepass");
        } else {
          check(p_bvq_fakequant_bwd_stats(&d, gy.data_ptr(), x.data_ptr(), scale.data_ptr(), zp.data_ptr(),
                                          stat.data_ptr(), dx.data_ptr(), ds.data_ptr<float>(), sdt, qr[2], sdt,
                                          ws.data_ptr(), wsb, st),
                "bvq_fakequant_bwd_stats");
        }
      }
    } else {
      const int64_t wsb = p_bvq_fakequant_bwd_workspace_bytes(&d);
      if (wsb < 0) throw std::runtime_error("bvq_fakequant_bwd_workspace_bytes failed");
      at::Tensor ws = at::empty({wsb > 8 ? wsb : 8}, x.options().dtype(at::kByte));
      at::Tensor ds = at::empty({1}, x.options().dtype(at::kFloat));
      at::Tensor info = at::empty({p_bvq_tie_info_bytes(1) / 8}, x.options().dtype(at::kLong));
      check(p_bvq_fakequant_bwd(&d, gy.data_ptr(), x.data_ptr(), scale.data_ptr(), zp.data_ptr(), dx.data_ptr(),
                                ds.data_ptr<float>(), nullptr, stat.data_ptr(), info.data_ptr<int64_t>(), ws.data_ptr(), ws.numel(),
                                st),
            "bvq_fakequant_bwd");
      const int64_t* total_ties = nullptr;
      at::Tensor total;
      if (group) {
        const int rank = group->getRank(), world = group->getSize();
        at::Tensor msg = at::empty({2}, x.options().dtype(at::kDouble));
        check(p_bvq_shard_pack(ds.data_ptr<float>(), info.data_ptr<int64_t>(), 1, rank, 0, msg.data_ptr<double>(), st),
              "bvq_shard_pack");
        at::Tensor gathered = at::empty({world * msg.numel()}, msg.options());
        if (const NativeComm* nc = native_comm(group->getGroupName())) {
          rccl_check(rccl().all_gather(msg.data_ptr<double>(), gathered.data_ptr<double>(), (size_t)msg.numel(),
                                       ncclFloat64, nc->comm, reinterpret_cast<hipStream_t>(st)),
                     "ncclAllGather");
        } else {
          group->_allgather_base(gathered, msg)->wait();
        }
        total = at::empty({1}, x.options().dtype(at::kLong));
        check(p_bvq_shard_unpack(gathered.data_ptr<double>(), world, 1, rank, 0, ds.data_ptr<float>(),
                                 info.data_ptr<int64_t>(), total.data_ptr<int64_t>(), st),
              "bvq_shard_unpack");
        total_ties = total.data_ptr<int64_t>();
      }
      check(p_bvq_stat_tie_apply_dscale(d.pre_op, d.x_dtype, x.data_ptr(), stat.data_ptr(), ds.data_ptr<float>(), sdt,
                                        qr[2], (int)dv[17], info.data_ptr<int64_t>(), total_ties, dx.data_ptr(), d.outer,
                                        d.channels, d.inner, st),
            "bvq_stat_tie_apply_dscale");
    }
    out[0] = dx;
    return out;
  }
};

Params make_params(const std::vector<int64_t>& di, double qmin, double qmax, double min_val, bool has_min, double thr_fwd,
                   double thr_bwd, double thr_raw, int64_t scale_dtype, std::vector<int64_t> shape, int64_t stream) {
  Params p;
  std::vector<double> qr{qmin, qmax};
  p.d = desc_from(di, qr);
  p.min_val = min_val;
  p.has_min = has_min ? 1 : 0;
  p.thr_fwd = thr_fwd;
  p.thr_bwd = thr_bwd;
  p.thr_raw = thr_raw;
  p.scale_dtype = (int)scale_dtype;
  p.stream = stream;
  p.shape = std::move(shape);
  return p;
}

}

void init(const std::string& lib_path, py::object fallback) {
  void* h = dlopen(lib_path.c_str(), RTLD_NOW | RTLD_GLOBAL);
  if (!h) throw std::runtime_error(std::string("dlopen ") + lib_path + ": " + dlerror());
#define BVQ_RESOLVE(name)                                                                      \
  p_##name = reinterpret_cast<decltype(&name)>(dlsym(h, #name));                               \
  if (!p_##name) throw std::runtime_error(std::string("libbvq.so: missing entry point ") + #name);
  BVQ_ENTRIES(BVQ_RESOLVE)
#undef BVQ_RESOLVE
  const int ver = p_bvq_abi_version();
  if (ver != BVQ_ABI_VERSION)
// ... 105 lines not shown
```

### brevitas_amd/csrc/bvq_fakequant_fwd.hip

```cpp

#include "bvq_fakequant.h"

namespace bvq {

template <typename CT, int RM, bool ZP0, typename Div>
__device__ __forceinline__ float fwd_elem(float xf, const Div& div, float s, float z, float qmin,
                                          float qmax, bool out_int, int mode, float& q_out) {
  float t = rnd<CT>(div(xf));
  t = ZP0 ? t + 0.f : rnd<CT>(t + z);
  t = do_round<CT, RM>(t, mode);
  const float q = clamp_where(t, qmin, qmax);
  q_out = q;
  if (out_int) return q;
  return ZP0 ? rnd<CT>(q * s) : rnd<CT>(rnd<CT>(q - z) * s);
}

template <typename CT, int RM, bool ZP0, typename Div, typename S>
__device__ __forceinline__ f2 fwd_elem2(f2 xf, const Div& div, S s, S z, float qmin, float qmax,
                                        bool out_int, int mode, f2& q_out) {
  f2 t = rnd2<CT>(div(xf));
  t = ZP0 ? t + 0.f : rnd2<CT>(t + z);
  t = do_round2<CT, RM>(t, mode);
  const f2 q = clamp_where2(t, qmin, qmax);
  q_out = q;
  if (out_int) return q;
  return ZP0 ? q * s : rnd2<CT>(q - z) * s;
}

template <int VEC>
__device__ __forceinline__ void store_codes(void* base, int codes_dtype, int64_t off, const float* q) {
  if (codes_dtype == BVQ_CODES_I32) {
    vec_t<int32_t, VEC> cv;
#pragma unroll
    for (int k = 0; k < VEC; ++k) cv.v[k] = (int32_t)q[k];
    store_vec<int32_t, VEC>(reinterpret_cast<int32_t*>(base) + off, cv);
  } else if (codes_dtype == BVQ_CODES_I8) {
    vec_t<int8_t, VEC> cv;
#pragma unroll
    for (int k = 0; k < VEC; ++k) cv.v[k] = (int8_t)(int32_t)q[k];
    store_vec<int8_t, VEC>(reinterpret_cast<int8_t*>(base) + off, cv);
  } else {
    vec_t<uint8_t, VEC> cv;
#pragma unroll
    for (int k = 0; k < VEC; ++k) cv.v[k] = (uint8_t)(int32_t)q[k];
    store_vec<uint8_t, VEC>(reinterpret_cast<uint8_t*>(base) + off, cv);
  }
}

template <typename XT, typename CT, int VEC, int RM, bool NT, bool ZP0, bool PRE, bool NTL = NT, typename Div>
__device__ __forceinline__ void fwd_unit(const QuantArgs& a, const Unit& u, const Div& div, float s,
                                         float z, float qmin, float qmax) {
  const int lane = threadIdx.x & 63;
  const XT* __restrict__ xp = reinterpret_cast<const XT*>(a.x) + u.base;
  CT* __restrict__ yp = a.y ? reinterpret_cast<CT*>(a.y) + u.base : nullptr;
  void* const cp = a.codes;
  const bool out_int = a.out_int != 0;
  const int mode = a.round_mode;

  ChunkCursor cur;
  cur.init(u, VEC, lane);
  const int64_t total = (int64_t)u.nrows * cur.cpr;
  for (int64_t done = 0; done < total; done += (int64_t)kWave * kUnroll) {
    vec_t<XT, VEC> xv[kUnroll];
    int64_t off[kUnroll];
    bool ok[kUnroll];
#pragma unroll
    for (int j = 0; j < kUnroll; ++j) {
      ok[j] = cur.valid();
      off[j] = cur.offset(u.row_stride, VEC);
      xv[j] = load_vec<XT, VEC, NTL>(xp + (ok[j] ? off[j] : 0));
      cur.next();
    }
#pragma unroll
    for (int j = 0; j < kUnroll; ++j) {
      if (ok[j]) {
        vec_t<CT, VEC> yv;
        float qv[VEC];
        if constexpr (VEC % 2 == 0) {
#pragma unroll
          for (int k = 0; k < VEC; k += 2) {
            f2 xf = widen2<XT>(xv[j].v[k], xv[j].v[k + 1]);
            if constexpr (PRE) xf = relu2(xf);
            f2 q2;
            const f2 r = fwd_elem2<CT, RM, ZP0>(xf, div, s, z, qmin, qmax, out_int, mode, q2);
            pack2<CT>(r, yv.v[k], yv.v[k + 1]);
            qv[k] = q2.x;
            qv[k + 1] = q2.y;
          }
        } else {
#pragma unroll
          for (int k = 0; k < VEC; ++k) {
            const float xf = PRE ? relu_f(to_f<XT>(xv[j].v[k])) : to_f<XT>(xv[j].v[k]);
            const float r = fwd_elem<CT, RM, ZP0>(xf, div, s, z, qmin, qmax, out_int, mode, qv[k]);
            yv.v[k] = from_f<CT>(r);
          }
        }
        if (yp) store_vec<CT, VEC, NT>(yp + off[j], yv);
        if (cp) store_codes<VEC>(cp, a.codes_dtype, u.base + off[j], qv);
      }
    }
  }
  const int32_t tail = (int32_t)(u.len - (int64_t)cur.cpr * VEC);
  for (int32_t e = lane; e < u.nrows * tail; e += kWave) {
    const int32_t tr = e / tail, tk = e - tr * tail;
    const int64_t i = (int64_t)tr * u.row_stride + (int64_t)cur.cpr * VEC + tk;
    float q;
    const float xf = PRE ? relu_f(to_f<XT>(xp[i])) : to_f<XT>(xp[i]);
    const float r = fwd_elem<CT, RM, ZP0>(xf, div, s, z, qmin, qmax, out_int, mode, q);
    if (yp) yp[i] = from_f<CT>(r);
    if (cp) store_codes<1>(cp, a.codes_dtype, u.base + i, &q);
  }
}

template <typename XT, typename CT, int VEC, int RM, bool NT, bool NTL = NT>
__global__ __launch_bounds__(kBlock) void fakequant_fwd_kernel(QuantArgs a) {
  const Unit u = locate_unit(a.t);
  if (!u.valid) return;
  float s, z;
  load_scale_zp<CT>(a, u.channel, s, z);
  const float qmin = rnd<CT>(a.bounds ? a.bounds[0] : a.qmin), qmax = rnd<CT>(a.bounds ? a.bounds[1] : a.qmax);
  const bool zp0 = sizeof(CT) == 2 && zp_is_pos_zero(z);
#define BVQ_FWD_UNIT(ZP0, PRE, DIV) fwd_unit<XT, CT, VEC, RM, NT, ZP0, PRE, NTL>(a, u, DIV, s, z, qmin, qmax)
#define BVQ_FWD_PRE(ZP0, DIV)      \
  do {                             \
    if (a.pre_relu)                \
      BVQ_FWD_UNIT(ZP0, true, DIV); \
    else                           \
      BVQ_FWD_UNIT(ZP0, false, DIV); \
  } while (0)
  if constexpr (elem<CT>::id == BVQ_BF16) {
    if (bf16_scale_ok(s)) {
      const DivBf16 div{1.0f / s};
      if (zp0)
        BVQ_FWD_PRE(true, div);
      else
        BVQ_FWD_PRE(false, div);
      return;
    }
  }
#ifndef BVQ_F16_FWD_EXACT
  if constexpr (elem<CT>::id == BVQ_F16) {
    if (f16_scale_ok(s)) {
      const DivF16R div{s, 1.0f / s};
      if (zp0)
        BVQ_FWD_PRE(true, div);
      else
        BVQ_FWD_PRE(false, div);
      return;
    }
  }
#endif
  const DivExact div{s};
  if constexpr (sizeof(CT) == 2) {
    if (zp0) {
// ... 24 lines not shown
  const buf_t by = make_buf(reinterpret_cast<T*>(a.y) + ln.blk0 * a.p.L, bytes);
  const uint32_t step = (uint32_t)((int64_t)a.p.rpp * a.p.L * (int64_t)sizeof(T));
  uint32_t off = (uint32_t)(((int64_t)ln.sub * a.p.L + (int64_t)ln.chunk * VEC) * (int64_t)sizeof(T));
  const int32_t steps = (int32_t)((nrows + a.p.rpp - 1) / a.p.rpp);
  f2 r2[VEC / 2];
#pragma unroll
  for (int k = 0; k < VEC / 2; ++k) r2[k] = f2{1.0f / ln.s2[k].x, 1.0f / ln.s2[k].y};
  const int mode = a.round_mode;
  for (int32_t i = 0; i < steps; i += kU) {
    vec_t<T, VEC> xv[kU];
#pragma unroll
    for (int j = 0; j < kU; ++j) xv[j] = buf_load<T, VEC, NT>(bx, off + (uint32_t)j * step);
#pragma unroll
    for (int j = 0; j < kU; ++j) {
      if (i + j < steps) {
        vec_t<T, VEC> yv;
#pragma unroll
        for (int k = 0; k < VEC; k += 2) {
          f2 xf = widen2<T>(xv[j].v[k], xv[j].v[k + 1]);
          if constexpr (PRE) xf = relu2(xf);
          f2 q2, res;
          if constexpr (FAST && elem<T>::id == BVQ_F16)
            res = fwd_elem2<T, RM, ZP0>(xf, BVQ_DIVF16V{ln.s2[k / 2], r2[k / 2]}, ln.s2[k / 2], ln.z2[k / 2], qmin, qmax, false,
                                        mode, q2);
          else if constexpr (FAST)
            res = fwd_elem2<T, RM, ZP0>(xf, DivBf16V{r2[k / 2]}, ln.s2[k / 2], ln.z2[k / 2], qmin, qmax, false, mode, q2);
          else
            res = fwd_elem2<T, RM, ZP0>(xf, DivExactV{ln.s2[k / 2]}, ln.s2[k / 2], ln.z2[k / 2], qmin, qmax, false, mode, q2);
          pack2<T>(res, yv.v[k], yv.v[k + 1]);
        }
        buf_store<T, VEC, NT>(by, off + (uint32_t)j * step, yv);
      }
    }
    off += (uint32_t)kU * step;
  }
}

template <typename T, int RM, bool NT>
__global__ __launch_bounds__(kBlock) void fakequant_fwd_cols_kernel(ColsQuantArgs a) {
  ColsLane<T, kColsFwdVec<T>> ln;
  if (!ln.init(a) || !ln.active) return;
  const float qmin = rnd<T>(a.qmin), qmax = rnd<T>(a.qmax);
#define BVQ_COLS_FWD(ZP0, FAST)                                \
  do {                                                         \
    if (a.pre_relu)                                            \
      cols_fwd_rows<T, RM, NT, ZP0, FAST, true>(a, ln, qmin, qmax);  \
    else                                                       \
      cols_fwd_rows<T, RM, NT, ZP0, FAST, false>(a, ln, qmin, qmax); \
  } while (0)
  if constexpr (sizeof(T) == 2) {
    if (ln.fast) {
      if (ln.zp0)
        BVQ_COLS_FWD(true, true);
      else
        BVQ_COLS_FWD(false, true);
      return;
    }
    if (ln.zp0) {
      BVQ_COLS_FWD(true, false);
      return;
    }
  }
  BVQ_COLS_FWD(false, false);
#undef BVQ_COLS_FWD
}

constexpr int kFusedSlots = 8;
constexpr int kFusedSliceChunks = 512;
constexpr int kFusedMaxWaves = 8;

struct FusedArgs {
  const void* x;
  void* y;
  void* stat_out;
  void* scale_out;
  int64_t outer, inner;
  int32_t channels;
  int32_t cpr;
  int32_t spr;
  int32_t slices;
  float qmin, qmax, min_val, int_threshold;
  int32_t use_min, scale_dtype, scale_pc, scalar_cast, round_mode, pre_relu;
};

template <typename T>
__device__ __forceinline__ float scale_from_key(uint32_t key, bool use_min, float min_val, float int_threshold,
                                                int scale_dtype, float& stat) {
  if constexpr (elem<T>::id == BVQ_F16)
    stat = (float)__builtin_bit_cast(f16_t, (uint16_t)key);
  else
    stat = __builtin_bit_cast(float, key);
  const float thr = (use_min && stat < min_val) ? min_val : stat;
  float s = thr / int_threshold;
  if (scale_dtype == BVQ_BF16)
    s = rnd<bf16_t>(s);
  else if (scale_dtype == BVQ_F16)
    s = rnd<f16_t>(s);
  return s;
}
template <typename T>
__device__ __forceinline__ void store_stat_scale(void* stat_out, void* scale_out, int scale_dtype, int32_t c,
                                                 float stat, float s) {
  if constexpr (elem<T>::id == BVQ_F32)
    reinterpret_cast<float*>(stat_out)[c] = stat;
  else
    reinterpret_cast<T*>(stat_out)[c] = (T)stat;
  if (scale_dtype == BVQ_F32)
    reinterpret_cast<float*>(scale_out)[c] = s;
  else if (scale_dtype == BVQ_BF16)
    reinterpret_cast<bf16_t*>(scale_out)[c] = (bf16_t)s;
  else
    reinterpret_cast<f16_t*>(scale_out)[c] = (f16_t)s;
}

template <typename T, int RM, bool PRE, typename Div>
__device__ __forceinline__ void fused_quantize(const vec_t<T, elem<T>::vec> (&xv)[kFusedSlots], const bool (&ok)[kFusedSlots],
                                               T* __restrict__ yp, int lane, const Div& div, float s,
                                               float qmin, float qmax, int mode) {
  constexpr int VEC = elem<T>::vec;
  constexpr bool ZP0 = sizeof(T) == 2;
#pragma unroll
  for (int j = 0; j < kFusedSlots; ++j) {
    if (ok[j]) {
      vec_t<T, VEC> yv;
#pragma unroll
      for (int k = 0; k < VEC; k += 2) {
        f2 xf = widen2<T>(xv[j].v[k], xv[j].v[k + 1]);
        if constexpr (PRE) xf = relu2(xf);
        f2 q2;
        const f2 r = fwd_elem2<T, RM, ZP0>(xf, div, s, 0.f, qmin, qmax, false, mode, q2);
        pack2<T>(r, yv.v[k], yv.v[k + 1]);
      }
      store_vec<T, VEC, true>(yp + (int64_t)(lane + kWave * j) * VEC, yv);
    }
  }
}

__global__ void fused_zero_kernel(uint32_t* p, int64_t n) {
  const int64_t i = (int64_t)blockIdx.x * blockDim.x + threadIdx.x;
  if (i < n) p[i] = 0u;
}

__device__ __forceinline__ void fused_slice(const FusedArgs& a, int q, int lane, int& r, int& sl, bool (&ok)[kFusedSlots]) {
  const bool active = q < a.slices;
  r = active ? q / a.spr : 0;
  sl = active ? q - r * a.spr : 0;
  const int nch = active ? (a.cpr - sl * kFusedSliceChunks < kFusedSliceChunks ? a.cpr - sl * kFusedSliceChunks
                                                                              : kFusedSliceChunks)
                         : 0;
#pragma unroll
  for (int j = 0; j < kFusedSlots; ++j) ok[j] = lane + kWave * j < nch;
}

template <typename T, int RM>
__device__ __forceinline__ void fused_channel(const FusedArgs& a, int32_t c, int r, int sl, const bool (&ok)[kFusedSlots],
                                              float qmin, float qmax, int wave, int lane, int nwaves,
                                              uint32_t* sh_max, uint32_t& sh_stat) {
  constexpr int VEC = elem<T>::vec;
  const int64_t base = ((int64_t)r * a.channels + c) * a.inner + (int64_t)sl * kFusedSliceChunks * VEC;
  const T* __restrict__ xp = reinterpret_cast<const T*>(a.x) + base;
  T* __restrict__ yp = reinterpret_cast<T*>(a.y) + base;
  vec_t<T, VEC> xv[kFusedSlots];
#pragma unroll
  for (int j = 0; j < kFusedSlots; ++j)
    xv[j] = load_vec<T, VEC, true>(ok[j] ? xp + (int64_t)(lane + kWave * j) * VEC : reinterpret_cast<const T*>(a.x));
  uint32_t m = 0;
#pragma unroll
  for (int j = 0; j < kFusedSlots; ++j) {
    if (ok[j]) {
#pragma unroll
      for (int k = 0; k < VEC; ++k) {
        const uint32_t b = a.pre_relu ? pre_abs_bits<T, true>(xv[j].v[k]) : pre_abs_bits<T, false>(xv[j].v[k]);
        m = b > m ? b : m;
      }
    }
  }
  m = wave_max_u32(m);
  if (lane == 0) sh_max[wave] = m;
  __syncthreads();
  if (threadIdx.x == 0) {
    uint32_t bm = 0;
    for (int w = 0; w < nwaves; ++w) bm = sh_max[w] > bm ? sh_max[w] : bm;
    sh_stat = bm;
  }
  __syncthreads();
  float stat;
  float s = scale_from_key<T>(sh_stat, a.use_min, a.min_val, a.int_threshold, a.scale_dtype, stat);
  if (threadIdx.x == 0) store_stat_scale<T>(a.stat_out, a.scale_out, a.scale_dtype, c, stat, s);
  if (a.scalar_cast && !a.scale_pc) s = rnd<T>(s);
  const int mode = a.round_mode;
  if constexpr (elem<T>::id == BVQ_BF16) {
    if (bf16_scale_ok(s)) {
      const DivBf16 div{1.0f / s};
      if (a.pre_relu)
        fused_quantize<T, RM, true>(xv, ok, yp, lane, div, s, qmin, qmax, mode);
      else
        fused_quantize<T, RM, false>(xv, ok, yp, lane, div, s, qmin, qmax, mode);
      return;
    }
  }
  if constexpr (elem<T>::id == BVQ_F16) {
    if (f16_scale_ok(s)) {
      const DivF16R div{s, 1.0f / s};
      if (a.pre_relu)
        fused_quantize<T, RM, true>(xv, ok, yp, lane, div, s, qmin, qmax, mode);
      else
        fused_quantize<T, RM, false>(xv, ok, yp, lane, div, s, qmin, qmax, mode);
      return;
    }
  }
  const DivExact div{s};
  if (a.pre_relu)
    fused_quantize<T, RM, true>(xv, ok, yp, lane, div, s, qmin, qmax, mode);
  else
    fused_quantize<T, RM, false>(xv, ok, yp, lane, div, s, qmin, qmax, mode);
}

template <typename T, int RM>
__global__ __launch_bounds__(kFusedMaxWaves * kWave) void fused_absmax_fakequant_kernel(FusedArgs a) {
  __shared__ uint32_t sh_max[kFusedMaxWaves];
  __shared__ uint32_t sh_stat;
  const int lane = threadIdx.x & 63;
  const int wave = __builtin_amdgcn_readfirstlane((int)(threadIdx.x >> 6));
  const int nwaves = (int)(blockDim.x >> 6);
  int r, sl;
  bool ok[kFusedSlots];
  fused_slice(a, wave, lane, r, sl, ok);
  const float qmin = rnd<T>(a.qmin), qmax = rnd<T>(a.qmax);
  for (int32_t c = blockIdx.x; c < a.channels; c += gridDim.x)
    fused_channel<T, RM>(a, c, r, sl, ok, qmin, qmax, wave, lane, nwaves, sh_max, sh_stat);
}

struct FusedListArgs {
  FusedArgs a[BVQ_WEIGHT_LIST_MAX];
  int32_t start[BVQ_WEIGHT_LIST_MAX + 1];
  int32_t n;
};
static_assert(sizeof(FusedListArgs) <= 4096, "kernel arguments are limited to 4 KiB");

template <typename T, int RM>
__global__ __launch_bounds__(kFusedMaxWaves * kWave) void fused_list_fakequant_kernel(FusedListArgs la) {
  __shared__ uint32_t sh_max[kFusedMaxWaves];
  __shared__ uint32_t sh_stat;
  const int lane = threadIdx.x & 63;
  const int wave = __builtin_amdgcn_readfirstlane((int)(threadIdx.x >> 6));
  const int nwaves = (int)(blockDim.x >> 6);
  int p = -1, r = 0, sl = 0;
  bool ok[kFusedSlots];
  float qmin = 0.f, qmax = 0.f;
  for (int32_t pair = blockIdx.x; pair < la.start[la.n]; pair += gridDim.x) {
    if (p < 0 || pair >= la.start[p + 1]) {
      if (p < 0) p = 0;
      while (p + 1 < la.n && pair >= la.start[p + 1]) ++p;
      fused_slice(la.a[p], wave, lane, r, sl, ok);
      qmin = rnd<T>(la.a[p].qmin);
      qmax = rnd<T>(la.a[p].qmax);
    }
    fused_channel<T, RM>(la.a[p], pair - la.start[p], r, sl, ok, qmin, qmax, wave, lane, nwaves, sh_max, sh_stat);
  }
}

}

using namespace bvq;

static int fakequant_fwd_impl(const bvq_quant_desc* d, const void* x, const void* scale, const void* zp, void* y,
                             void* codes, const float* bounds, bvq_stream_t stream) {
  int rc = validate(d);
  if (rc) return rc;
  const int64_t n = d->outer * d->channels * d->inner;
  if (n == 0) return BVQ_OK;
  if (!x || !scale || !zp || (!y && !codes)) {
    set_error("bvq_fakequant_fwd: null pointer");
    return BVQ_ERR_INVALID;
  }
  if (y && !codes && !bounds) {
    const ColsPlan cp = cols_quant_plan(d, x, y, nullptr, true, false, kColsFwdVec16);
    if (cp.ok) {
      ColsQuantArgs ca = {};
      fill_cols_args(ca, cp, d);
      ca.x = x;
      ca.y = y;
      ca.scale = scale;
      ca.zp = zp;
      hipStream_t cst = (hipStream_t)stream;
      const bool cnt = n * (int64_t)(2 * dtype_size(d->x_dtype)) >= nt_threshold_bytes();
      rc = with_cols_variant(d, cnt, [&](auto t, auto rm, auto ntc) {
        fakequant_fwd_cols_kernel<typename decltype(t)::type, rm, ntc><<<grid_for_units(cp.units), kBlock, 0, cst>>>(ca);
      });
      return rc ? rc : check_launch("bvq_fakequant_fwd/cols");
    }
  }
  int64_t outer, row_len;
  int32_t channels;
  rows_of(d, outer, row_len, channels);
  const void* ptrs[3] = {x, y, codes};
  const int els[3] = {dtype_size(d->x_dtype), dtype_size(d->ct_dtype), d->codes_dtype == BVQ_CODES_I32 ? 4 : 1};
  const int full = 16 / dtype_size(d->x_dtype);
  const int vec = snap_vec(pick_vec(full, outer * channels, row_len, ptrs, els, 3, true), full);
  QuantArgs a = {};
  a.t = make_tiling(outer, channels, row_len, vec, 0, true);
  a.x = x;
  a.scale = scale;
  a.zp = zp;
  a.y = y;
  a.codes = codes;
  a.bounds = bounds;
  fill_args(a, d);
  hipStream_t st = (hipStream_t)stream;
  const bool nt = n * (int64_t)(dtype_size(d->x_dtype) + dtype_size(d->ct_dtype)) >= nt_threshold_bytes();
  rc = with_pair(d->x_dtype, d->ct_dtype, [&](auto xt, auto ct) {
    using XT = typename decltype(xt)::type;
    return with_stream_variant<elem<XT>::vec>("bvq_fakequant_fwd", vec, a.round_mode, nt, [&](auto v, auto rm, auto ntc) {
      fakequant_fwd_kernel<XT, typename decltype(ct)::type, v, rm, ntc><<<grid_for_units(a.t.units), kBlock, 0, st>>>(a);
    });
  });
  return rc ? rc : check_launch("bvq_fakequant_fwd");
}

extern "C" int bvq_fakequant_fwd(const bvq_quant_desc* d, const void* x, const void* scale,
                                 const void* zp, void* y, void* codes, bvq_stream_t stream) {
  return fakequant_fwd_impl(d, x, scale, zp, y, codes, nullptr, stream);
}

extern "C" int bvq_fakequant_fwd_bounds(const bvq_quant_desc* d, const void* x, const void* scale, const void* zp,
                                        const float* bounds, void* y, bvq_stream_t stream) {
  if (!bounds) {
    set_error("bvq_fakequant_fwd_bounds: null bounds");
    return BVQ_ERR_INVALID;
  }
  return fakequant_fwd_impl(d, x, scale, zp, y, nullptr, bounds, stream);
}


struct FusedPlan {
  int32_t cpr, spr, slices, waves, nblocks;
};

static int num_cus() {
  static int n = [] {
    int dev = 0, v = 0;
    if (hipGetDevice(&dev) != hipSuccess ||
        hipDeviceGetAttribute(&v, hipDeviceAttributeMultiprocessorCount, dev) != hipSuccess || v <= 0)
      v = 256;
    return v;
  }();
  return n;
}

struct FusedShape {
  bool ok;
  int64_t outer, channels, inner;
  int vec;
};

#ifndef BVQ_FUSED_FWD
#define BVQ_FUSED_FWD 1
#endif
constexpr bool kFusedFwd = BVQ_FUSED_FWD != 0;

static FusedShape fused_shape(const bvq_quant_desc* d, const void* x, const void* y) {
  FusedShape f = {};
  if (!kFusedFwd) return f;
  if (d->x_dtype != d->ct_dtype || d->out_kind != BVQ_OUT_DEQUANT) return f;
  if (d->zp_per_channel) return f;
  const bool pc = d->scale_per_channel && d->channels > 1;
  f.outer = pc ? d->outer : 1;
  f.channels = pc ? d->channels : 1;
  f.inner = pc ? d->inner : d->outer * d->channels * d->inner;
  f.vec = 16 / dtype_size(d->x_dtype);
  if (f.inner <= 0 || f.outer <= 0 || f.inner % f.vec != 0) return f;
  if ((reinterpret_cast<uintptr_t>(x) | reinterpret_cast<uintptr_t>(y)) & 15) return f;
  f.ok = true;
  return f;
}

static bool fused_plan(const bvq_quant_desc* d, const void* x, const void* y, FusedPlan& p) {
  const FusedShape f = fused_shape(d, x, y);
  if (!f.ok) return false;
  const int64_t cpr = f.inner / f.vec;
  const int64_t spr = (cpr + kFusedSliceChunks - 1) / kFusedSliceChunks;
  const int64_t slices = f.outer * spr;
  if (cpr > (1 << 30) || slices > kFusedMaxWaves) return false;
  p.cpr = (int32_t)cpr;
  p.spr = (int32_t)spr;
  p.slices = (int32_t)slices;
  p.waves = (int)slices;
  const int64_t budget = (int64_t)num_cus() * 2 * kFusedMaxWaves / p.waves;
  p.nblocks = (int32_t)(budget < f.channels ? budget : f.channels);
  return true;
}

extern "C" int64_t bvq_stats_fakequant_fwd_workspace_bytes(const bvq_quant_desc* d, const void* x, const void* y) {
  if (validate(d)) return -1;
  FusedPlan p;
  if (fused_plan(d, x, y, p)) return 16;
  return 0;
}

static FusedArgs fused_args(const bvq_quant_desc* d, const FusedPlan& p, const void* x, void* y, void* stat_out,
                            void* scale_out, double min_val, int use_min, double int_threshold) {
  const bool pc = d->scale_per_channel && d->channels > 1;
  FusedArgs a = {};
  a.x = x;
  a.y = y;
  a.stat_out = stat_out;
  a.scale_out = scale_out;
  a.outer = pc ? d->outer : 1;
  a.inner = pc ? d->inner : d->outer * d->channels * d->inner;
  a.channels = (int32_t)(pc ? d->channels : 1);
  a.cpr = p.cpr;
  a.spr = p.spr;
  a.slices = p.slices;
  a.qmin = d->qmin;
  a.qmax = d->qmax;
  a.min_val = round_host((float)min_val, d->x_dtype);
  a.use_min = use_min;
  a.int_threshold = (float)int_threshold;
  a.scale_dtype = d->scale_dtype;
  a.scale_pc = pc ? 1 : 0;
  a.scalar_cast = d->scalar_mode == BVQ_SCALAR_CAST;
  a.round_mode = d->round_mode;
  a.pre_relu = d->pre_op == BVQ_PRE_RELU;
  return a;
}

extern "C" int bvq_stats_fakequant_fwd(const bvq_quant_desc* d, const void* x, double min_val, int use_min,
                                       double int_threshold, void* stat_out, void* scale_out, void* y,
                                       void* workspace, int64_t workspace_bytes, bvq_stream_t stream) {
  int rc = validate(d);
  if (rc) return rc;
  if (!x || !y || !stat_out || !scale_out || !workspace) {
    set_error("bvq_stats_fakequant_fwd: null pointer");
    return BVQ_ERR_INVALID;
  }
  hipStream_t st = (hipStream_t)stream;
  FusedPlan p;
  if (fused_plan(d, x, y, p)) {
    const FusedArgs a = fused_args(d, p, x, y, stat_out, scale_out, min_val, use_min, int_threshold);
    const dim3 grid((unsigned)p.nblocks), block((unsigned)(p.waves * kWave));
    rc = with_cols_variant(d, false, [&](auto t, auto rm, auto) {
      fused_absmax_fakequant_kernel<typename decltype(t)::type, rm><<<grid, block, 0, st>>>(a);
    });
    return rc ? rc : check_launch("bvq_stats_fakequant_fwd");
  }
  set_error("bvq_stats_fakequant_fwd: shape / layout not covered by the one-launch form");
  return BVQ_ERR_UNSUPPORTED;
}

namespace bvq {
int fused_list_fwd(int n, const bvq_quant_desc* descs, const bvq_weight_item* items, hipStream_t st) {
  FusedListArgs la = {};
  la.n = n;
  int64_t pairs = 0;
  int waves = 1;
  for (int i = 0; i < n; ++i) {
    const bvq_weight_item& it = items[i];
    FusedPlan p;
    if (!fused_plan(&descs[i], it.x, it.y, p)) {
      set_error("bvq_weight_quant_list_fwd: item %d not covered by the one-launch form", i);
      return BVQ_ERR_UNSUPPORTED;
    }
    la.a[i] = fused_args(&descs[i], p, it.x, it.y, it.stat, it.scale, it.min_val, it.use_min, it.int_threshold);
    la.start[i] = (int32_t)pairs;
    pairs += la.a[i].channels;
    waves = p.waves > waves ? p.waves : waves;
  }
  if (pairs >= ((int64_t)1 << 31)) {
    set_error("bvq_weight_quant_list_fwd: too many channels");
    return BVQ_ERR_UNSUPPORTED;
  }
  la.start[n] = (int32_t)pairs;
  const int64_t budget = (int64_t)num_cus() * 2 * kFusedMaxWaves / waves;
  const dim3 grid((unsigned)(budget < pairs ? budget : pairs)), block((unsigned)(waves * kWave));
  const int rc = with_cols_variant(&descs[0], false, [&](auto t, auto rm, auto) {
    fused_list_fakequant_kernel<typename decltype(t)::type, rm><<<grid, block, 0, st>>>(la);
  });
  return rc ? rc : check_launch("bvq_weight_quant_list_fwd");
}
}

__global__ __launch_bounds__(256) void selftest_div_f16r_kernel(const float* __restrict__ a, const float* __restrict__ sc,
                                                                float* __restrict__ out, int32_t n_a) {
  const float s = sc[blockIdx.y];
  const float r = 1.0f / s;
  for (int32_t i = blockIdx.x * 256 + threadIdx.x; i < n_a; i += gridDim.x * 256)
    out[(int64_t)blockIdx.y * n_a + i] = div_refined(a[i], s, r);
}

extern "C" int bvq_selftest_div_f16r(const float* a, int32_t n_a, const float* scales, int32_t n_s, float* out,
                                     bvq_stream_t stream) {
  if (!a || !scales || !out || n_a < 1 || n_s < 1 || n_s > 65535) {
    set_error("bvq_selftest_div_f16r: bad argument");
    return BVQ_ERR_INVALID;
  }
  int nb = (n_a + 255) / 256;
  if (nb > 1024) nb = 1024;
  selftest_div_f16r_kernel<<<dim3((unsigned)nb, (unsigned)n_s), dim3(256), 0, (hipStream_t)stream>>>(a, scales, out, n_a);
  return check_launch("bvq_selftest_div_f16r");
}
```

### brevitas_amd/csrc/bvq_stats.hip

```cpp
#include <math.h>
#include <string.h>

#include "bvq_common.h"
#include "bvq_ties.h"
#include "bvq_sums.h"

namespace bvq {

constexpr int kStatUnroll = 8;

struct StatArgs {
  Tiling t;
  const void* x;
  uint32_t* part_a;
  uint32_t* part_b;
  float* pivot;
};

template <typename T, int VEC, bool NT, bool RELU>
__global__ __launch_bounds__(kBlock) void absmax_kernel(StatArgs a) {
  const Unit u = locate_unit(a.t);
  if (!u.valid) return;
  const int lane = threadIdx.x & 63;
  const T* __restrict__ xp = reinterpret_cast<const T*>(a.x) + u.base;
  uint32_t m = 0;
  ChunkWalker cur;
  cur.init(u, VEC, lane);
  const int64_t total = (int64_t)u.nrows * cur.cpr;
  for (int64_t done = 0; done < total; done += (int64_t)kWave * kStatUnroll) {
    vec_t<T, VEC> xv[kStatUnroll];
    bool ok[kStatUnroll];
#pragma unroll
    for (int j = 0; j < kStatUnroll; ++j) {
      ok[j] = cur.valid();
      if (ok[j]) xv[j] = load_vec<T, VEC, NT>(xp + cur.offset(u.row_stride, VEC));
      cur.next();
    }
#pragma unroll
    for (int j = 0; j < kStatUnroll; ++j) {
      if (ok[j]) {
#pragma unroll
        for (int k = 0; k < VEC; ++k) {
          const uint32_t b = pre_abs_bits<T, RELU>(xv[j].v[k]);
          m = b > m ? b : m;
        }
      }
    }
  }
  const int32_t tail = (int32_t)(u.len - (int64_t)cur.cpr * VEC);
  for (int32_t e = lane; e < u.nrows * tail; e += kWave) {
    const int32_t r = e / tail, k = e - r * tail;
    const uint32_t b = pre_abs_bits<T, RELU>(xp[(int64_t)r * u.row_stride + (int64_t)cur.cpr * VEC + k]);
    m = b > m ? b : m;
  }
  m = wave_max_u32(m);
  if (lane == 0) a.part_a[u.id] = m;
}

template <typename T, int VEC, bool NT, bool RELU>
__global__ __launch_bounds__(kBlock) void minmax_kernel(StatArgs a) {
  const Unit u = locate_unit(a.t);
  if (!u.valid) return;
  const int lane = threadIdx.x & 63;
  const T* __restrict__ xp = reinterpret_cast<const T*>(a.x) + u.base;
  float mx = -__builtin_inff(), mn = __builtin_inff();
  uint32_t nan = 0;
  ChunkWalker cur;
  cur.init(u, VEC, lane);
  const int64_t total = (int64_t)u.nrows * cur.cpr;
  for (int64_t done = 0; done < total; done += (int64_t)kWave * kStatUnroll) {
    vec_t<T, VEC> xv[kStatUnroll];
    bool ok[kStatUnroll];
#pragma unroll
    for (int j = 0; j < kStatUnroll; ++j) {
      ok[j] = cur.valid();
      if (ok[j]) xv[j] = load_vec<T, VEC, NT>(xp + cur.offset(u.row_stride, VEC));
      cur.next();
    }
#pragma unroll
    for (int j = 0; j < kStatUnroll; ++j) {
      if (ok[j]) {
#pragma unroll
        for (int k = 0; k < VEC; ++k) {
          const float f = RELU ? relu_f(to_f<T>(xv[j].v[k])) : to_f<T>(xv[j].v[k]);
          nan |= (f != f) ? 1u : 0u;
          mx = fmaxf(mx, f);
          mn = fminf(mn, f);
        }
      }
    }
  }
  const int32_t tail = (int32_t)(u.len - (int64_t)cur.cpr * VEC);
  for (int32_t e = lane; e < u.nrows * tail; e += kWave) {
    const int32_t r = e / tail, k = e - r * tail;
    const T xe = xp[(int64_t)r * u.row_stride + (int64_t)cur.cpr * VEC + k];
    const float f = RELU ? relu_f(to_f<T>(xe)) : to_f<T>(xe);
    nan |= (f != f) ? 1u : 0u;
    mx = fmaxf(mx, f);
    mn = fminf(mn, f);
  }
  mx = wave_max(mx);
  mn = wave_min(mn);
  nan = wave_or_u32(nan);
  if (lane == 0) {
    a.part_a[u.id] = nan ? 0x7fc00000u : __builtin_bit_cast(uint32_t, mx);
    a.part_b[u.id] = nan ? 0x7fc00000u : __builtin_bit_cast(uint32_t, mn);
  }
}

template <typename T>
__device__ __forceinline__ float moments_pivot(const void* x, int64_t first) {
  const float p = fabsf(to_f<T>(reinterpret_cast<const T*>(x)[first]));
  return p <= 3.4028234663852886e38f ? p : 0.f;
}

template <typename T, int VEC, bool NT>
__global__ __launch_bounds__(kBlock) void absmoments_kernel(StatArgs a) {
  const Unit u = locate_unit(a.t);
  if (!u.valid) return;
  const int lane = threadIdx.x & 63;
  const T* __restrict__ xp = reinterpret_cast<const T*>(a.x) + u.base;
  const float p = moments_pivot<T>(a.x, (int64_t)u.channel * a.t.row_len);
  float s1 = 0.f, s2 = 0.f;
  ChunkWalker cur;
  cur.init(u, VEC, lane);
  const int64_t total = (int64_t)u.nrows * cur.cpr;
  for (int64_t done = 0; done < total; done += (int64_t)kWave * kStatUnroll) {
    vec_t<T, VEC> xv[kStatUnroll];
    bool ok[kStatUnroll];
#pragma unroll
    for (int j = 0; j < kStatUnroll; ++j) {
      ok[j] = cur.valid();
      if (ok[j]) xv[j] = load_vec<T, VEC, NT>(xp + cur.offset(u.row_stride, VEC));
      cur.next();
    }
#pragma unroll
    for (int j = 0; j < kStatUnroll; ++j) {
      if (ok[j]) {
#pragma unroll
        for (int k = 0; k < VEC; ++k) {
          const float d = fabsf(to_f<T>(xv[j].v[k])) - p;
          s1 += d;
          s2 += d * d;
        }
      }
    }
  }
  const int64_t i = (int64_t)cur.cpr * VEC + lane;
  if (u.nrows == 1 && i < u.len) {
    const float d = fabsf(to_f<T>(xp[i])) - p;
    s1 += d;
    s2 += d * d;
  }
  s1 = wave_sum(s1);
  s2 = wave_sum(s2);
  if (lane == 0) {
    a.part_a[u.id] = __builtin_bit_cast(uint32_t, s1);
    a.part_b[u.id] = __builtin_bit_cast(uint32_t, s2);
// ... 28 lines not shown
      store_vec<T, VEC>(dp + off, dv);
    }
    cur.next();
  }
  if (u.nrows == 1 && lane == 0) {
    for (int64_t e = (int64_t)cur.cpr * VEC; e < u.len; ++e) dp[e] = f(xp[e]);
  }
}

template <typename T>
__global__ __launch_bounds__(kBlock) void abs_affine_bwd_cols_kernel(const void* x, const float* ca, const float* cb,
                                                                     void* dx, int64_t rows, int64_t L, int64_t inner) {
  constexpr int VEC = elem<T>::vec;
  const int64_t cc = (int64_t)blockIdx.x * kBlock + threadIdx.x;
  if (cc * VEC >= L) return;
  float a[VEC], b[VEC];
#pragma unroll
  for (int k = 0; k < VEC; ++k) {
    const int64_t c = (cc * VEC + k) / inner;
    a[k] = ca[c];
    b[k] = cb[c];
  }
  const T* __restrict__ xp = reinterpret_cast<const T*>(x) + cc * VEC;
  T* __restrict__ dp = reinterpret_cast<T*>(dx) + cc * VEC;
  for (int64_t r = blockIdx.y; r < rows; r += gridDim.y) {
    const vec_t<T, VEC> xv = load_vec<T, VEC>(xp + r * L);
    vec_t<T, VEC> dv;
#pragma unroll
    for (int k = 0; k < VEC; ++k) {
      const float xf = to_f<T>(xv.v[k]);
      const float m = a[k] + b[k] * fabsf(xf);
      dv.v[k] = from_f<T>(xf > 0.f ? m : (xf < 0.f ? -m : (xf == 0.f ? 0.f : xf)));
    }
    store_vec<T, VEC>(dp + r * L, dv);
  }
}

struct ColsStatArgs {
  ColsPlan p;
  const void* x;
  uint32_t* part;
};

template <typename T, bool NT, bool RELU>
__global__ __launch_bounds__(kBlock) void absmax_cols_kernel(ColsStatArgs a) {
  constexpr int VEC = elem<T>::vec;
  const int wave = __builtin_amdgcn_readfirstlane((int)(threadIdx.x >> 6));
  const int lane = threadIdx.x & 63;
  const int64_t unit = (int64_t)blockIdx.x * kWavesPerBlock + wave;
  if (unit >= a.p.units) return;
  const int64_t rblk = unit / a.p.strips;
  const int32_t strip = (int32_t)(unit - rblk * a.p.strips);
  const int32_t sub = lane / a.p.lpr;
  const int32_t chunk = strip * kWave + (lane - sub * a.p.lpr);
  const bool active = sub < a.p.rpp && chunk < a.p.cps;
  const int64_t row0 = rblk * a.p.rb + sub;
  const int64_t row_end = (rblk + 1) * a.p.rb < a.p.rows ? (rblk + 1) * a.p.rb : a.p.rows;
  const T* __restrict__ xp = reinterpret_cast<const T*>(a.x) + (int64_t)chunk * VEC;
  uint32_t m[VEC];
#pragma unroll
  for (int k = 0; k < VEC; ++k) m[k] = 0;
  if (active) {
    constexpr int kU = 4;
    for (int64_t r = row0; r < row_end; r += (int64_t)kU * a.p.rpp) {
      vec_t<T, VEC> xv[kU];
      bool ok[kU];
#pragma unroll
      for (int j = 0; j < kU; ++j) {
        const int64_t rr = r + (int64_t)j * a.p.rpp;
        ok[j] = rr < row_end;
        xv[j] = load_vec<T, VEC, NT>(xp + (ok[j] ? rr : row0) * a.p.L);
      }
#pragma unroll
      for (int j = 0; j < kU; ++j) {
        if (ok[j]) {
#pragma unroll
          for (int k = 0; k < VEC; ++k) {
            const uint32_t b = pre_abs_bits<T, RELU>(xv[j].v[k]);
            m[k] = b > m[k] ? b : m[k];
          }
        }
      }
    }
    uint32_t* out = a.part + (rblk * a.p.rpp + sub) * a.p.L + (int64_t)chunk * VEC;
#pragma unroll
    for (int k = 0; k < VEC; ++k) out[k] = m[k];
  }
}

struct ColsMomentArgs {
  ColsPlan p;
  const void* x;
  float* part1;
  float* part2;
  float* pivot;
  int64_t inner;
};

template <typename T, bool NT>
__global__ __launch_bounds__(kBlock) void absmoments_cols_kernel(ColsMomentArgs a) {
  constexpr int VEC = elem<T>::vec;
  const int wave = __builtin_amdgcn_readfirstlane((int)(threadIdx.x >> 6));
  const int lane = threadIdx.x & 63;
  const int64_t unit = (int64_t)blockIdx.x * kWavesPerBlock + wave;
  if (unit >= a.p.units) return;
  const int64_t rblk = unit / a.p.strips;
  const int32_t strip = (int32_t)(unit - rblk * a.p.strips);
  const int32_t sub = lane / a.p.lpr;
  const int32_t chunk = strip * kWave + (lane - sub * a.p.lpr);
  const bool active = sub < a.p.rpp && chunk < a.p.cps;
  if (!active) return;
  const int64_t row0 = rblk * a.p.rb + sub;
  const int64_t row_end = (rblk + 1) * a.p.rb < a.p.rows ? (rblk + 1) * a.p.rb : a.p.rows;
  const T* __restrict__ xp = reinterpret_cast<const T*>(a.x) + (int64_t)chunk * VEC;
  float pv[VEC], s1[VEC], s2[VEC];
#pragma unroll
  for (int k = 0; k < VEC; ++k) {
    const int64_t col = (int64_t)chunk * VEC + k;
    const int64_t c = col / a.inner;
    pv[k] = moments_pivot<T>(a.x, c * a.inner);
    s1[k] = s2[k] = 0.f;
    if (rblk == 0 && sub == 0 && col == c * a.inner) a.pivot[c] = pv[k];
  }
  constexpr int kU = 4;
  for (int64_t r = row0; r < row_end; r += (int64_t)kU * a.p.rpp) {
    vec_t<T, VEC> xv[kU];
    bool ok[kU];
#pragma unroll
    for (int j = 0; j < kU; ++j) {
      const int64_t rr = r + (int64_t)j * a.p.rpp;
      ok[j] = rr < row_end;
      xv[j] = load_vec<T, VEC, NT>(xp + (ok[j] ? rr : row0) * a.p.L);
    }
#pragma unroll
    for (int j = 0; j < kU; ++j) {
      if (ok[j]) {
#pragma unroll
        for (int k = 0; k < VEC; ++k) {
          const float d = fabsf(to_f<T>(xv[j].v[k])) - pv[k];
          s1[k] += d;
          s2[k] += d * d;
        }
      }
    }
  }
  const int64_t base = (rblk * a.p.rpp + sub) * a.p.L + (int64_t)chunk * VEC;
#pragma unroll
  for (int k = 0; k < VEC; ++k) {
    a.part1[base + k] = s1[k];
    a.part2[base + k] = s2[k];
  }
}

__device__ __forceinline__ void store_stat(void* out, int out_dtype, int64_t idx, float v) {
  if (out_dtype == BVQ_F32)
    reinterpret_cast<float*>(out)[idx] = v;
  else if (out_dtype == BVQ_BF16)
    reinterpret_cast<bf16_t*>(out)[idx] = (bf16_t)v;
  else
    reinterpret_cast<f16_t*>(out)[idx] = (f16_t)v;
}

__device__ __forceinline__ uint32_t order_key(float f) {
  const uint32_t u = __builtin_bit_cast(uint32_t, f);
  return (u >> 31) ? ~u : (u | 0x80000000u);
}

__device__ __forceinline__ float order_key_value(uint32_t k) {
  return __builtin_bit_cast(float, (k >> 31) ? (k ^ 0x80000000u) : ~k);
}

template <typename T, bool NT, bool RELU>
__global__ __launch_bounds__(kBlock) void minmax_cols_kernel(ColsStatArgs a) {
  constexpr int VEC = elem<T>::vec;
  const int wave = __builtin_amdgcn_readfirstlane((int)(threadIdx.x >> 6));
  const int lane = threadIdx.x & 63;
  const int64_t unit = (int64_t)blockIdx.x * kWavesPerBlock + wave;
  if (unit >= a.p.units) return;
  const int64_t rblk = unit / a.p.strips;
  const int32_t strip = (int32_t)(unit - rblk * a.p.strips);
  const int32_t sub = lane / a.p.lpr;
  const int32_t chunk = strip * kWave + (lane - sub * a.p.lpr);
  const bool active = sub < a.p.rpp && chunk < a.p.cps;
  const int64_t row0 = rblk * a.p.rb + sub;
  const int64_t row_end = (rblk + 1) * a.p.rb < a.p.rows ? (rblk + 1) * a.p.rb : a.p.rows;
  const T* __restrict__ xp = reinterpret_cast<const T*>(a.x) + (int64_t)chunk * VEC;
  float mx[VEC], mn[VEC];
  uint32_t nan = 0;
#pragma unroll
  for (int k = 0; k < VEC; ++k) {
    mx[k] = -__builtin_inff();
    mn[k] = __builtin_inff();
  }
  if (active) {
    constexpr int kU = 4;
    for (int64_t r = row0; r < row_end; r += (int64_t)kU * a.p.rpp) {
      vec_t<T, VEC> xv[kU];
      bool ok[kU];
#pragma unroll
      for (int j = 0; j < kU; ++j) {
        const int64_t rr = r + (int64_t)j * a.p.rpp;
        ok[j] = rr < row_end;
        xv[j] = load_vec<T, VEC, NT>(xp + (ok[j] ? rr : row0) * a.p.L);
      }
#pragma unroll
      for (int j = 0; j < kU; ++j) {
        if (ok[j]) {
#pragma unroll
          for (int k = 0; k < VEC; ++k) {
            const float f = RELU ? relu_f(to_f<T>(xv[j].v[k])) : to_f<T>(xv[j].v[k]);
            nan |= (f != f) ? (1u << k) : 0u;
            mx[k] = fmaxf(mx[k], f);
            mn[k] = fminf(mn[k], f);
          }
        }
      }
    }
    uint32_t* out = a.part + (rblk * a.p.rpp + sub) * (2 * a.p.L) + (int64_t)chunk * VEC;
#pragma unroll
    for (int k = 0; k < VEC; ++k) {
      const bool bad = (nan >> k) & 1u;
      out[k] = bad ? 0xffffffffu : order_key(mx[k]);
      out[a.p.L + k] = bad ? 0xffffffffu : order_key(-mn[k]);
    }
  }
}

__global__ __launch_bounds__(kWave) void minmax_cols_finish_kernel(const uint32_t* __restrict__ folded, void* out,
                                                                   int out_dtype, int32_t channels, int64_t inner) {
  const int32_t c = blockIdx.x;
  const int64_t L = (int64_t)channels * inner;
  uint32_t kx = 0, kn = 0;
  for (int64_t i = threadIdx.x; i < inner; i += kWave) {
    const uint32_t a = folded[(int64_t)c * inner + i], b = folded[L + (int64_t)c * inner + i];
    kx = a > kx ? a : kx;
    kn = b > kn ? b : kn;
  }
  kx = wave_max_u32(kx);
  kn = wave_max_u32(kn);
  if (threadIdx.x == 0) {
    const bool bad = kx == 0xffffffffu || kn == 0xffffffffu;
    const float qn = __builtin_nanf("");
    store_stat(out, out_dtype, c, bad ? qn : order_key_value(kx));
    store_stat(out, out_dtype, (int64_t)channels + c, bad ? qn : -order_key_value(kn));
  }
}

struct ScaleEpilogue {
  void* scale_out;
  int32_t scale_dtype;
  int32_t use_min;
  float min_val;
  float int_threshold;
  void* running;
  int32_t run_dtype, first_batch;
  float momentum, one_minus_m;
};

__device__ __forceinline__ float running_update(float r, float o, int run_dtype, int stat_dtype, float one_minus_m,
                                                float m, int first) {
  auto round_to = [](float v, int dt) {
    return dt == BVQ_F32 ? v : (dt == BVQ_BF16 ? rnd<bf16_t>(v) : rnd<f16_t>(v));
  };
  if (first) return round_to(r * o, run_dtype);
  r = round_to(r * one_minus_m, run_dtype);
  const float u = round_to(o * m, stat_dtype);
  return round_to(r + u, run_dtype);
}

constexpr int64_t kFinishSlice = 4096;

static inline int32_t finish_splits(int64_t partials_per_channel) {
  const int64_t s = (partials_per_channel + kFinishSlice - 1) / kFinishSlice;
  return (int32_t)(s < 1 ? 1 : s);
}

template <int KIND>
__global__ __launch_bounds__(kBlock) void stat_finish_kernel(const uint32_t* __restrict__ part_a,
                                                             const uint32_t* __restrict__ part_b,
                                                             void* out, int out_dtype, int in_dtype,
                                                             int64_t nob, int32_t channels,
                                                             int64_t ppr, ScaleEpilogue ep,
                                                             uint32_t* __restrict__ mid_a,
                                                             uint32_t* __restrict__ mid_b) {
  __shared__ uint32_t sha[kBlock];
  __shared__ float shx[kBlock], shn[kBlock];
  __shared__ uint32_t shnan[kBlock];
  const int32_t c = blockIdx.x;
  const int64_t n = nob * ppr;
  const int64_t slice = (n + gridDim.y - 1) / gridDim.y;
  const int64_t k0 = (int64_t)blockIdx.y * slice;
  const int64_t k1 = k0 + slice < n ? k0 + slice : n;
  uint32_t m = 0;
  float mx = -__builtin_inff(), mn = __builtin_inff();
  uint32_t nan = 0;
  for (int64_t k = k0 + threadIdx.x; k < k1; k += kBlock) {
    int64_t unit;
    if (nob == 1) {
      unit = (int64_t)c * ppr + k;
    } else {
      const int64_t o = k / ppr, p = k - o * ppr;
      unit = (o * channels + c) * ppr + p;
    }
    if (KIND == BVQ_STAT_ABSMAX) {
      const uint32_t b = part_a[unit];
      m = b > m ? b : m;
    } else {
      const float a = __builtin_bit_cast(float, part_a[unit]);
      const float b = __builtin_bit_cast(float, part_b[unit]);
      nan |= (a != a) ? 1u : 0u;
      mx = fmaxf(mx, a);
      mn = fminf(mn, b);
    }
  }
  sha[threadIdx.x] = m;
  shx[threadIdx.x] = mx;
  shn[threadIdx.x] = mn;
  shnan[threadIdx.x] = nan;
  __syncthreads();
  for (int st = kBlock / 2; st > 0; st >>= 1) {
    if ((int)threadIdx.x < st) {
      const uint32_t o = sha[threadIdx.x + st];
      if (o > sha[threadIdx.x]) sha[threadIdx.x] = o;
      shx[threadIdx.x] = fmaxf(shx[threadIdx.x], shx[threadIdx.x + st]);
      shn[threadIdx.x] = fminf(shn[threadIdx.x], shn[threadIdx.x + st]);
      shnan[threadIdx.x] |= shnan[threadIdx.x + st];
    }
    __syncthreads();
  }
  if (threadIdx.x == 0 && mid_a) {
    const int64_t slot = (int64_t)c * gridDim.y + blockIdx.y;
    if (KIND == BVQ_STAT_ABSMAX) {
      mid_a[slot] = sha[0];
    } else {
      mid_a[slot] = shnan[0] ? 0x7fc00000u : __builtin_bit_cast(uint32_t, shx[0]);
      mid_b[slot] = __builtin_bit_cast(uint32_t, shn[0]);
    }
  } else if (threadIdx.x == 0) {
    if (KIND == BVQ_STAT_ABSMAX) {
      float v;
      if (in_dtype == BVQ_F16) {
        v = (float)__builtin_bit_cast(f16_t, (uint16_t)sha[0]);
      } else {
        v = __builtin_bit_cast(float, sha[0]);
      }
      store_stat(out, out_dtype, c, v);
      if (ep.scale_out) {
        const float thr = (ep.use_min && v < ep.min_val) ? ep.min_val : v;
        store_stat(ep.scale_out, ep.scale_dtype, c, thr / ep.int_threshold);
      }
      if (ep.running) {
        const float r = load_scalar_as_f(ep.running, ep.run_dtype, c);
        store_stat(ep.running, ep.run_dtype, c,
                   running_update(r, v, ep.run_dtype, out_dtype, ep.one_minus_m, ep.momentum, ep.first_batch));
      }
    } else {
      const float qn = __builtin_nanf("");
      store_stat(out, out_dtype, c, shnan[0] ? qn : shx[0]);
      store_stat(out, out_dtype, (int64_t)channels + c, shnan[0] ? qn : shn[0]);
    }
  }
}

struct ArriveArgs {
  uint32_t* key;
  uint32_t* cnt;
  uint32_t per_channel;
  void* stat_out;
  int32_t stat_dtype, in_dtype;
  uint32_t* part;
};

__device__ __forceinline__ bool arrive_max(uint32_t* key, uint32_t* cnt, uint32_t m, uint32_t n, uint32_t expected,
                                           uint32_t& out) {
  const uint32_t seen = __hip_atomic_fetch_max(key, m, __ATOMIC_RELAXED, __HIP_MEMORY_SCOPE_AGENT);
  uint32_t add = n;
  asm volatile("" : "+v"(add) : "v"(seen));
  const uint32_t before = __hip_atomic_fetch_add(cnt, add, __ATOMIC_RELAXED, __HIP_MEMORY_SCOPE_AGENT);
  if (before + add != expected) return false;
  out = __hip_atomic_exchange(key, 0u, __ATOMIC_RELAXED, __HIP_MEMORY_SCOPE_AGENT);
  __hip_atomic_store(cnt, 0u, __ATOMIC_RELAXED, __HIP_MEMORY_SCOPE_AGENT);
  return true;
}

__device__ __forceinline__ void absmax_finish(const ArriveArgs& r, const ScaleEpilogue& ep, int32_t c, uint32_t bits) {
  const float v = r.in_dtype == BVQ_F16 ? (float)__builtin_bit_cast(f16_t, (uint16_t)bits)
                                         : __builtin_bit_cast(float, bits);
  store_stat(r.stat_out, r.stat_dtype, c, v);
  if (ep.scale_out) {
    const float thr = (ep.use_min && v < ep.min_val) ? ep.min_val : v;
    store_stat(ep.scale_out, ep.scale_dtype, c, thr / ep.int_threshold);
  }
  if (ep.running) {
    const float run = load_scalar_as_f(ep.running, ep.run_dtype, c);
    store_stat(ep.running, ep.run_dtype, c,
               running_update(run, v, ep.run_dtype, r.stat_dtype, ep.one_minus_m, ep.momentum, ep.first_batch));
  }
}

__device__ __forceinline__ void absmax_arrive(const ArriveArgs& r, const ScaleEpilogue& ep, int32_t c, uint32_t m,
                                              uint32_t n, int lane) {
  m = wave_max_u32(m);
  if (lane != 0) return;
  uint32_t bits;
  if (arrive_max(r.key + c, r.cnt + c, m, n, r.per_channel, bits)) absmax_finish(r, ep, c, bits);
}

constexpr int kOnepassDepth = 4;

template <typename T, int VEC, bool NT, bool RELU>
__device__ __forceinline__ uint32_t onepass_unit_max(const StatArgs& a, const Unit& u, int lane) {
  const T* __restrict__ xp = reinterpret_cast<const T*>(a.x) + u.base;
  const int64_t extent = (int64_t)(u.nrows - 1) * u.row_stride + u.len;
  const buf_t bx = make_buf(xp, (uint32_t)(extent * (int64_t)sizeof(T)));
  constexpr uint32_t kSkip = 0x60000000u;
  constexpr int kD = kOnepassDepth;
  ChunkCursor cur;
  cur.init(u, VEC, lane);
  const int64_t total = (int64_t)u.nrows * cur.cpr;
  const int32_t steps = (int32_t)((total + kWave - 1) / kWave);
  const uint32_t rs = (uint32_t)u.row_stride;
  uint32_t m = 0;
  typedef unsigned short u16x2 __attribute__((ext_vector_type(2)));
  u16x2 m2 = {0, 0};
  auto fold = [&](const vec_t<T, VEC>& xv) {
    if constexpr (sizeof(T) == 2 && VEC % 2 == 0 && !RELU) {
      const vec_t<uint32_t, VEC / 2> w = __builtin_bit_cast(vec_t<uint32_t, VEC / 2>, xv);
#pragma unroll
      for (int k = 0; k < VEC / 2; ++k)
        m2 = __builtin_elementwise_max(m2, __builtin_bit_cast(u16x2, w.v[k] & 0x7fff7fffu));
    } else {
#pragma unroll
      for (int k = 0; k < VEC; ++k) {
        const uint32_t b = pre_abs_bits<T, RELU>(xv.v[k]);
        m = b > m ? b : m;
      }
    }
  };
  vec_t<T, VEC> xb[kD];
#pragma unroll
  for (int j = 0; j < kD; ++j) {
    const uint32_t off = cur.valid() ? cur.offset32(rs, VEC) : kSkip;
    xb[j] = buf_load<T, VEC, NT>(bx, off * (uint32_t)sizeof(T));
    cur.next();
  }
  for (int32_t base = 0; base < steps; base += kD) {
#pragma unroll
    for (int j = 0; j < kD; ++j) {
      if (base + j >= steps) break;
      fold(xb[j]);
      const uint32_t off = cur.valid() ? cur.offset32(rs, VEC) : kSkip;
      xb[j] = buf_load<T, VEC, NT>(bx, off * (uint32_t)sizeof(T));
      cur.next();
    }
  }
  if constexpr (sizeof(T) == 2 && VEC % 2 == 0 && !RELU) {
    const uint32_t m16 = m2.x > m2.y ? m2.x : m2.y;
    m = elem<T>::id == BVQ_BF16 ? (m16 << 16) : m16;
  }
  const int32_t tail = (int32_t)(u.len - (int64_t)cur.cpr * VEC);
  for (int32_t e = lane; e < u.nrows * tail; e += kWave) {
    const int32_t tr = e / tail, k = e - tr * tail;
    const uint32_t b = pre_abs_bits<T, RELU>(xp[(int64_t)tr * u.row_stride + (int64_t)cur.cpr * VEC + k]);
    m = b > m ? b : m;
  }
  return m;
}

template <typename T, int VEC, bool NT, bool RELU>
__global__ __launch_bounds__(kBlock) void absmax_onepass_kernel(StatArgs a, ArriveArgs r, ScaleEpilogue ep) {
  const Unit u = locate_unit(a.t);
  if (!u.valid) return;
  const int lane = threadIdx.x & 63;
  uint32_t m = onepass_unit_max<T, VEC, NT, RELU>(a, u, lane);
  if (r.part) {
    m = wave_max_u32(m);
    if (lane == 0) r.part[u.id] = m;
    return;
  }
  absmax_arrive(r, ep, u.channel, m, 1u, lane);
}


__global__ void shard_pack_kernel(const float* __restrict__ ds, const long long* __restrict__ tie_info,
                                  double* __restrict__ out, int32_t channels, int32_t rank, int per_channel) {
  const int c = blockIdx.x * blockDim.x + threadIdx.x;
  if (c >= channels) return;
  out[c] = (double)ds[c];
  if (per_channel)
    out[channels + c] = tie_info[c] >= 0 ? (double)rank : kShardNoOwner;
  else
    out[channels + c] = (double)tie_info[0];
}

__global__ void shard_unpack_kernel(const double* __restrict__ all, int32_t world, int32_t channels, int32_t rank,
                                    int per_channel, float* __restrict__ ds_total, long long* __restrict__ tie_info,
                                    long long* __restrict__ total_ties) {
  const int c = blockIdx.x * blockDim.x + threadIdx.x;
  if (c >= channels) return;
  double sum = 0.0, owner = kShardNoOwner, count = 0.0;
  for (int r = 0; r < world; ++r) {
    const double* m = all + (size_t)r * 2 * channels;
    sum += m[c];
    const double k = m[channels + c];
    owner = k < owner ? k : owner;
    count += k;
  }
  ds_total[c] = (float)sum;
  if (per_channel) {
    if (owner != (double)rank) tie_info[c] = -1;
  } else if (c == 0) {
    total_ties[0] = (long long)count;
  }
}

__global__ void scale_from_stat_kernel(const float* __restrict__ stat32, void* stat_out, int stat_dtype, ScaleEpilogue ep,
                                       int32_t channels) {
  const int c = blockIdx.x * blockDim.x + threadIdx.x;
  if (c >= channels) return;
  const float v = stat32[c];
  store_stat(stat_out, stat_dtype, c, v);
  const float thr = (ep.use_min && v < ep.min_val) ? ep.min_val : v;
  store_stat(ep.scale_out, ep.scale_dtype, c, thr / ep.int_threshold);
  if (ep.running) {
    const float r = load_scalar_as_f(ep.running, ep.run_dtype, c);
    store_stat(ep.running, ep.run_dtype, c,
               running_update(r, v, ep.run_dtype, stat_dtype, ep.one_minus_m, ep.momentum, ep.first_batch));
  }
}

__global__ void running_stats_kernel(void* running, int run_dtype, const void* stat, int stat_dtype,
                                     int64_t n, float one_minus_m, float m, int first) {
  const int64_t i = (int64_t)blockIdx.x * blockDim.x + threadIdx.x;
  if (i >= n) return;
  float r = load_scalar_as_f(running, run_dtype, i);
  const float o = load_scalar_as_f(stat, stat_dtype, i);
  r = running_update(r, o, run_dtype, stat_dtype, one_minus_m, m, first);
  store_stat(running, run_dtype, i, r);
}


template <typename T, int MATCH>
__device__ __forceinline__ bool is_tie(T v, T stat) {
  if constexpr (MATCH == BVQ_MATCH_ABS) {
    return abs_bits<T>(v) == abs_bits<T>(stat);
  } else {
    return to_f<T>(v) == to_f<T>(stat);
  }
}
template <typename T, int MATCH>
// ... 1100 lines not shown
```

### include/bvq.h

```cpp
#ifndef BVQ_H_
#define BVQ_H_

#include <stddef.h>
#include <stdint.h>

#ifdef __cplusplus
extern "C" {
#endif

#define BVQ_ABI_VERSION 2

typedef void* bvq_stream_t;

typedef enum bvq_status {
  BVQ_OK = 0,
  BVQ_ERR_INVALID = -1,
  BVQ_ERR_UNSUPPORTED = -2,
  BVQ_ERR_WORKSPACE = -3,
  BVQ_ERR_LAUNCH = -4
} bvq_status;

typedef enum bvq_dtype { BVQ_F32 = 0, BVQ_BF16 = 1, BVQ_F16 = 2 } bvq_dtype;

typedef enum bvq_round_mode {
// ... 36 lines not shown
  int32_t x_dtype;
  int32_t ct_dtype;
  int32_t scale_dtype;
  int32_t zp_dtype;
  int32_t scale_per_channel;
  int32_t zp_per_channel;
  float qmin;
  float qmax;
  int32_t round_mode;
  int32_t scalar_mode;
  int32_t clamp_ste;
  int32_t out_kind;
  int32_t pre_op;
  int32_t codes_dtype;
} bvq_quant_desc;


int bvq_abi_version(void);
const char* bvq_last_error(void);


int bvq_unary(int op, int dtype, const void* x, void* y, int64_t n, bvq_stream_t stream);

int bvq_scalar_clamp(int dtype, const void* x, void* y, int64_t n, double lo, int use_lo, double hi,
                     int use_hi, bvq_stream_t stream);

int bvq_tensor_clamp(int dtype, const void* x, const void* lo, const void* hi, int bounds_full, void* y,
                     int64_t n, bvq_stream_t stream);

int bvq_tensor_clamp_bwd(int dtype, const void* g, const void* x, const void* lo, const void* hi,
                         int bounds_full, void* dx, int64_t n, bvq_stream_t stream);

int bvq_abs_binary_sign_grad_bwd(int dtype, const void* g, const void* x, void* dx, int64_t n,
                                 bvq_stream_t stream);


int64_t bvq_stats_workspace_bytes(int kind, int dtype, int64_t outer, int64_t channels, int64_t inner);

int bvq_stats(int kind, int dtype, const void* x, int64_t outer, int64_t channels, int64_t inner,
              int out_dtype, void* out, void* workspace, int64_t workspace_bytes, bvq_stream_t stream);

int bvq_stats_pre(int kind, int pre_op, int dtype, const void* x, int64_t outer, int64_t channels,
                  int64_t inner, int out_dtype, void* out, void* workspace, int64_t workspace_bytes,
                  bvq_stream_t stream);

int bvq_absmax_scale(int pre_op, int dtype, const void* x, int64_t outer, int64_t channels, int64_t inner,
                     void* stat_out, double min_val, int use_min, double int_threshold, int scale_dtype,
                     void* scale_out, void* workspace, int64_t workspace_bytes, bvq_stream_t stream);
int bvq_absmax_scale_running(int pre_op, int dtype, const void* x, int64_t outer, int64_t channels, int64_t inner,
                             void* stat_out, double min_val, int use_min, double int_threshold, int scale_dtype,
                             void* scale_out, int run_dtype, void* running, double momentum, int first_batch,
                             void* workspace, int64_t workspace_bytes, bvq_stream_t stream);

int bvq_absmax_onepass_supported(int dtype, const void* x, int64_t outer, int64_t channels, int64_t inner);
int bvq_absmax_scale_onepass(int pre_op, int dtype, const void* x, int64_t outer, int64_t channels, int64_t inner,
                             int stat_dtype, void* stat_out, double min_val, int use_min, double int_threshold,
                             int scale_dtype, void* scale_out, int run_dtype, void* running, double momentum,
                             int first_batch, uint32_t* arrive, int64_t arrive_words, bvq_stream_t stream);

int bvq_absmax_list_supported(int dtype, int n, const void* const* xs, const int64_t* outers, int64_t channels,
                              const int64_t* inners);
int bvq_absmax_scale_list(int dtype, int n, const void* const* xs, const int64_t* outers, int64_t channels,
                          const int64_t* inners, void* stat_out, double min_val, int use_min, double int_threshold,
                          int scale_dtype, void* scale_out, uint32_t* arrive, int64_t arrive_words,
                          void* workspace, int64_t workspace_bytes, bvq_stream_t stream);

int bvq_running_stats_update(int run_dtype, void* running, int stat_dtype, const void* stat, int64_t n,
                             double momentum, int first_batch, bvq_stream_t stream);

int bvq_scale_from_stat(const float* stat32, int64_t channels, int stat_dtype, void* stat_out, double min_val,
                        int use_min, double int_threshold, int scale_dtype, void* scale_out, bvq_stream_t stream);
int bvq_scale_from_stat_running(const float* stat32, int64_t channels, int stat_dtype, void* stat_out, double min_val,
                                int use_min, double int_threshold, int scale_dtype, void* scale_out, int run_dtype,
                                void* running, double momentum, int first_batch, bvq_stream_t stream);
int bvq_fakequant_bwd_shard(const bvq_quant_desc* d, const void* g, const void* x, const void* scale, const void* zp,
                            const void* stat, void* dx, double* message, int64_t* first_pos, int rank, void* workspace,
                            int64_t workspace_bytes, uint32_t* arrive, int64_t arrive_words, bvq_stream_t stream);
int bvq_shard_unpack_deposit(int dtype, const void* x, void* dx, const double* gathered, int world, int64_t channels,
                             int rank, const int64_t* first_pos, int64_t inner, int scale_dtype, double int_threshold,
                             int quot_dtype, int pre_op, float* dscale_total, bvq_stream_t stream);
int bvq_shard_pack(const float* dscale, const int64_t* tie_info, int64_t channels, int rank, int per_channel,
                   double* message, bvq_stream_t stream);
int bvq_shard_unpack(const double* gathered, int world, int64_t channels, int rank, int per_channel,
                     float* dscale_total, int64_t* tie_info, int64_t* total_ties, bvq_stream_t stream);

int bvq_histc(int dtype, const void* x, int64_t n, const void* absmax, int bins, int32_t* counts,
              bvq_stream_t stream);

int64_t bvq_abs_moments_workspace_bytes(int dtype, int64_t outer, int64_t channels, int64_t inner);
int bvq_abs_moments(int dtype, const void* x, int64_t outer, int64_t channels, int64_t inner, float* sums,
                    void* workspace, int64_t workspace_bytes, bvq_stream_t stream);
int bvq_abs_affine_bwd(int dtype, const void* x, const float* a, const float* b, void* dx, int64_t outer,
                       int64_t channels, int64_t inner, bvq_stream_t stream);

int64_t bvq_kth_workspace_bytes(int dtype, int64_t outer, int64_t channels, int64_t inner);
int bvq_kth_value(int abs_key, int dtype, const void* x, int64_t outer, int64_t channels, int64_t inner,
                  int64_t k, void* out, void* workspace, int64_t workspace_bytes, bvq_stream_t stream);
int bvq_kth_pair(int abs_key, int dtype, const void* x, int64_t outer, int64_t channels, int64_t inner,
                 int64_t k_first, int64_t k_second, void* out, void* workspace, int64_t workspace_bytes,
                 bvq_stream_t stream);

typedef enum bvq_kth_rule { BVQ_KTH_EXPLICIT = 0, BVQ_KTH_HIGH = 1, BVQ_KTH_LOW = 2 } bvq_kth_rule;
int bvq_kth_passes(int dtype);
int64_t bvq_kth_hist_offset(int dtype, int64_t channels, int pass);
int bvq_kth_begin(int dtype, int64_t channels, int rule, int64_t k, double q, void* workspace,
                  int64_t workspace_bytes, bvq_stream_t stream);
int bvq_kth_hist(int abs_key, int dtype, const void* x, int64_t outer, int64_t channels, int64_t inner,
                 int pass, void* workspace, int64_t workspace_bytes, bvq_stream_t stream);
int bvq_kth_pick(int dtype, int64_t channels, int pass, int rule, double q, void* workspace,
                 int64_t workspace_bytes, bvq_stream_t stream);
int bvq_kth_finish(int abs_key, int dtype, int64_t channels, void* out, void* workspace,
                   int64_t workspace_bytes, bvq_stream_t stream);

int bvq_kthw_plan(int abs_key, int dtype, int pass, int64_t* hist_offset_bytes, int64_t* hist_words);
int bvq_kthw_begin(int abs_key, int dtype, void* workspace, int64_t workspace_bytes, bvq_stream_t stream);
int bvq_kthw_hist(int abs_key, int dtype, const void* x, int64_t n, int pass, void* workspace,
                  int64_t workspace_bytes, bvq_stream_t stream);
int bvq_kthw_pick(int abs_key, int dtype, int pass, int rule, int64_t k, double q, void* workspace,
                  int64_t workspace_bytes, bvq_stream_t stream);
int bvq_kthw_finish(int abs_key, int dtype, void* out, void* workspace, int64_t workspace_bytes,
                    bvq_stream_t stream);

typedef enum bvq_match_kind {
  BVQ_MATCH_ABS = 0,
  BVQ_MATCH_VALUE = 1,
  BVQ_MATCH_FIRST = 16
} bvq_match_kind;

int bvq_stat_bwd(int match, int dtype, const void* x, const void* stat, const void* gstat, void* dx,
                 int64_t outer, int64_t channels, int64_t inner, int mode_add, void* workspace,
                 int64_t workspace_bytes, bvq_stream_t stream);

int64_t bvq_tie_info_bytes(int64_t channels);
int bvq_stat_tie_scan(int match, int dtype, const void* x, const void* stat, int64_t outer,
                      int64_t channels, int64_t inner, void* dx_zero_fill, int64_t* tie_info,
                      bvq_stream_t stream);
int bvq_stat_tie_apply(int match, int pre_op, int dtype, const void* x, const void* stat,
                       const void* gstat, const int64_t* tie_info, const int64_t* total_ties, void* dx,
                       int64_t outer, int64_t channels, int64_t inner, int mode_add, bvq_stream_t stream);

int bvq_stat_tie_apply_dscale(int pre_op, int dtype, const void* x, const void* stat, const float* dscale,
                              int scale_dtype, double int_threshold, int quot_dtype,
                              const int64_t* tie_info, const int64_t* total_ties, void* dx, int64_t outer,
                              int64_t channels, int64_t inner, bvq_stream_t stream);


int bvq_fakequant_fwd(const bvq_quant_desc* desc, const void* x, const void* scale, const void* zp,
                      void* y, void* codes, bvq_stream_t stream);

int64_t bvq_stats_fakequant_fwd_workspace_bytes(const bvq_quant_desc* desc, const void* x, const void* y);
int bvq_stats_fakequant_fwd(const bvq_quant_desc* desc, const void* x, double min_val, int use_min,
                            double int_threshold, void* stat_out, void* scale_out, void* y, void* workspace,
                            int64_t workspace_bytes, bvq_stream_t stream);

int64_t bvq_fakequant_bwd_workspace_bytes(const bvq_quant_desc* desc);

int bvq_fakequant_bwd(const bvq_quant_desc* desc, const void* g, const void* x, const void* scale,
                      const void* zp, void* dx, float* dscale, float* dzp, const void* tie_stat,
                      int64_t* tie_info, void* workspace, int64_t workspace_bytes, bvq_stream_t stream);

int bvq_fakequant_fwd_bounds(const bvq_quant_desc* desc, const void* x, const void* scale, const void* zp,
                             const float* bounds, void* y, bvq_stream_t stream);
int bvq_fakequant_bwd_bounds(const bvq_quant_desc* desc, const void* g, const void* x, const void* scale,
                             const void* zp, const float* bounds, void* dx, float* dscale, float* dbounds,
                             void* workspace, int64_t workspace_bytes, bvq_stream_t stream);

int bvq_learned_scale(int value_dtype, const void* value, int64_t n, double min_val, int use_min,
                      double int_threshold, int scale_dtype, void* scale_out, bvq_stream_t stream);
int bvq_fakequant_bwd_learned(const bvq_quant_desc* desc, const void* g, const void* x, const void* scale,
                              const void* zp, void* dx, float* dscale, const void* value, int value_dtype,
                              double min_val, int use_min, double int_threshold, const void* gscale,
                              void* dvalue, void* workspace, int64_t workspace_bytes, bvq_stream_t stream);

int64_t bvq_fakequant_bwd_stats_workspace_bytes(const bvq_quant_desc* desc);
int bvq_fakequant_bwd_stats(const bvq_quant_desc* desc, const void* g, const void* x, const void* scale,
                            const void* zp, const void* stat, void* dx, float* dscale, int scale_dtype,
                            double int_threshold, int quot_dtype, void* workspace, int64_t workspace_bytes,
                            bvq_stream_t stream);

int bvq_fakequant_bwd_stats_onepass_supported(const bvq_quant_desc* d);
int bvq_fakequant_bwd_stats_onepass(const bvq_quant_desc* d, const void* g, const void* x, const void* scale,
                                    const void* zp, const void* stat, void* dx, float* dscale, int scale_dtype,
                                    double int_threshold, int quot_dtype, void* workspace, int64_t workspace_bytes,
                                    uint32_t* arrive, int64_t arrive_words, bvq_stream_t stream);

typedef enum bvq_variant_kind {
  BVQ_VAR_BINARY = 0, BVQ_VAR_CLAMPED_BINARY = 1, BVQ_VAR_TERNARY = 2, BVQ_VAR_DECOUPLED = 3, BVQ_VAR_TRUNC = 4
} bvq_variant_kind;
typedef struct bvq_variant_desc {
  int64_t outer, channels, inner;
  int32_t kind;
  int32_t x_dtype, ct_dtype, scale_dtype, zp_dtype;
  int32_t scale_per_channel;
  int32_t round_mode;
  int32_t clamp_ste;
  int32_t scalar_mode;
  float qmin, qmax;
  float threshold;
  float trunc_scale;
} bvq_variant_desc;
int bvq_variant_fwd(const bvq_variant_desc* desc, const void* x, const void* scale, const void* pre_scale,
                    const void* zp, const void* pre_zp, void* y, bvq_stream_t stream);
int64_t bvq_variant_bwd_workspace_bytes(const bvq_variant_desc* desc);
int bvq_variant_bwd(const bvq_variant_desc* desc, const void* g, const void* x, const void* scale,
                    const void* pre_scale, const void* zp, const void* pre_zp, void* dx, float* dscale,
                    float* dpre_scale, void* workspace, int64_t workspace_bytes, bvq_stream_t stream);

#define BVQ_WEIGHT_LIST_MAX 16
typedef struct bvq_weight_item {
  const void* x;
  void* y;
  void* stat;
  void* scale;
  const void* g;
  void* dx;
  float* dscale;
  int64_t channels;
  int64_t inner;
  double min_val;
  double int_threshold;
  float qmin;
  float qmax;
  int32_t use_min;
  int32_t clamp_ste;
} bvq_weight_item;
int bvq_weight_list_supported(int dtype, int round_mode, int n, const bvq_weight_item* items, int64_t arrive_words);
int bvq_weight_quant_list_fwd(int dtype, int scale_dtype, int round_mode, int n, const bvq_weight_item* items,
                              bvq_stream_t stream);
int64_t bvq_weight_quant_list_bwd_workspace_bytes(int dtype, int n, const bvq_weight_item* items);
int bvq_weight_quant_list_bwd(int dtype, int scale_dtype, int quot_dtype, int round_mode, int n,
                              const bvq_weight_item* items, void* workspace, int64_t workspace_bytes, uint32_t* arrive,
                              int64_t arrive_words, bvq_stream_t stream);

int bvq_selftest_div_f16r(const float* a, int32_t n_a, const float* scales, int32_t n_s, float* out,
                          bvq_stream_t stream);

#ifdef __cplusplus
}
#endif
#endif
```

Baseline: 515.1.

## Add cluster kernel fusing per-channel absmax stats with fake-quant forward

Adds a cluster kernel for per-channel absmax where several blocks cooperate on one channel. Each block keeps its slice of x in registers and publishes its partial max to a global arrival buffer, then spins with a time budget until all members of its cluster have arrived. The scale is then computed and the data is quantized without a second read of x. It also prefetches the next channel's slice while waiting, folds the running-stats update into the same kernel, and falls back to rereading the channel if the spin times out. The cost being removed is the separate stats pass plus the separate fakequant_fwd launch that reread x. In exchange the kernel relies on all cluster members being co-resident, adds spin-wait overhead, and needs an arrival workspace.

```diff
diff --git a/brevitas_amd/_native.py b/brevitas_amd/_native.py
--- a/brevitas_amd/_native.py
+++ b/brevitas_amd/_native.py
@@ -17,6 +17,7 @@
 MATCH_FIRST = 16
 PRE_NONE, PRE_RELU = 0, 1
 CODES_I32, CODES_I8, CODES_U8 = 0, 1, 2
+CLUSTER_FORCE_FALLBACK = 1
 _CODES_TORCH = {CODES_I32: torch.int32, CODES_I8: torch.int8, CODES_U8: torch.uint8}
 ABI_VERSION = 2
 
@@ -35,7 +36,8 @@
     'bvq_absmax_onepass_supported', 'bvq_absmax_scale_onepass', 'bvq_fakequant_bwd_stats_onepass_supported',
     'bvq_fakequant_bwd_stats_onepass', 'bvq_scale_from_stat_running', 'bvq_fakequant_bwd_shard',
     'bvq_shard_unpack_deposit', 'bvq_absmax_list_supported', 'bvq_absmax_scale_list', 'bvq_weight_list_supported',
-    'bvq_weight_quant_list_fwd', 'bvq_weight_quant_list_bwd_workspace_bytes', 'bvq_weight_quant_list_bwd')
+    'bvq_weight_quant_list_fwd', 'bvq_weight_quant_list_bwd_workspace_bytes', 'bvq_weight_quant_list_bwd',
+    'bvq_absmax_fakequant_cluster_supported', 'bvq_absmax_fakequant_cluster')
 
 
 class QuantDesc(ctypes.Structure):
@@ -149,6 +151,9 @@
         'bvq_weight_quant_list_fwd': (i32, [i32, i32, i32, i32, vp, vp]),
         'bvq_weight_quant_list_bwd_workspace_bytes': (i64, [i32, i32, vp]),
         'bvq_weight_quant_list_bwd': (i32, [i32, i32, i32, i32, i32, vp, vp, i64, vp, i64, vp]),
+        'bvq_absmax_fakequant_cluster_supported': (i64, [ctypes.POINTER(QuantDesc), vp, vp]),
+        'bvq_absmax_fakequant_cluster': (i32, [ctypes.POINTER(QuantDesc), vp, dbl, i32, dbl, vp, vp, i32, vp, dbl, i32, vp,
+                                               vp, i64, i32, vp, vp]),
         'bvq_fakequant_bwd_learned': (i32, [ctypes.POINTER(QuantDesc), vp, vp, vp, vp, vp, vp, vp, i32, dbl, i32, dbl, vp, vp, vp, i64, vp]),
     }
     for name, (res, args) in sig.items():
@@ -405,6 +410,33 @@
         check(lib.bvq_stats_fakequant_fwd(ctypes.byref(desc), ptr(x), float(min_val or 0.0), int(bool(min_val)),
                                           float(int_threshold), ptr(stat), ptr(scale), ptr(y), ptr(ws), wsb,
                                           stream_ptr(dev)), 'bvq_stats_fakequant_fwd')
+        if _timer is not None:
+            _timer.after('bvq_stats_fakequant_fwd')
+    return stat, scale, y
+
+
+def absmax_fakequant_cluster(desc, x, min_val, int_threshold, scale_dtype, running=None, momentum=0.0,
+                             first_batch=False, flags=0, fallbacks=None):
+    dev = require_device(x)
+    assert x.is_contiguous()
+    y = torch.empty_like(x)
+    words = int(lib.bvq_absmax_fakequant_cluster_supported(ctypes.byref(desc), ptr(x), ptr(y)))
+    if words <= 0:
+        return None
+    with _DeviceGuard(dev):
+        st = stream_ptr(dev)
+        arrive = arrival_buffer(dev, st, words)
+        if arrive is None:
+            return None
+        stat = torch.empty(desc.channels, dtype=x.dtype, device=dev)
+        scale = torch.empty(desc.channels, dtype=scale_dtype, device=dev)
+        if _timer is not None:
+            _timer.before('bvq_stats_fakequant_fwd')
+        check(lib.bvq_absmax_fakequant_cluster(
+            ctypes.byref(desc), ptr(x), float(min_val or 0.0), int(bool(min_val)), float(int_threshold), ptr(stat),
+            ptr(scale), dtype_code(running.dtype) if running is not None else 0, ptr(running), float(momentum),
+            int(first_batch), ptr(y), ptr(arrive), arrive.numel(), int(flags), ptr(fallbacks), st),
+            'bvq_absmax_fakequant_cluster')
         if _timer is not None:
             _timer.after('bvq_stats_fakequant_fwd')
     return stat, scale, y
diff --git a/brevitas_amd/core/quant/_fused.py b/brevitas_amd/core/quant/_fused.py
--- a/brevitas_amd/core/quant/_fused.py
+++ b/brevitas_amd/core/quant/_fused.py
@@ -358,6 +358,19 @@
                                  nat.dtype_code(zp.dtype), int(sp.channels > 1), 0, qmin, qmax, round_mode,
                                  scalar_mode(), int(clamp_ste), nat.OUT_DEQUANT, pre_op)
             fused = nat.stats_fakequant_fwd(desc, xc, sp.min_val, thr_div, scale_dtype)
+            if fused is None and len(sp.scaling_shape) > 0 and sp.channels > 1:
+                running = None
+                if runtime is not None:
+                    buf = runtime.running_stats
+                    if buf.is_cuda and buf.is_contiguous() and buf.numel() == sp.channels and buf.dtype in _FLOATS:
+                        running = buf
+                if runtime is None or running is not None:
+                    fused = nat.absmax_fakequant_cluster(
+                        desc, xc, sp.min_val, thr_div, scale_dtype, running,
+                        runtime.momentum if running is not None else 0.0,
+                        runtime.first_batch if running is not None else False)
+                    if fused is not None and running is not None:
+                        runtime.bvq_running_folded = True
         if fused is not None:
             stat, scale, y = fused
             scale = scale.view(sp.scaling_shape)
diff --git a/brevitas_amd/csrc/build.py b/brevitas_amd/csrc/build.py
--- a/brevitas_amd/csrc/build.py
+++ b/brevitas_amd/csrc/build.py
@@ -19,7 +19,7 @@
            ('bvq_fakequant_bwd_f16.hip', [], 'bvq_fakequant_bwd_f16.o'),
            ('bvq_fakequant_bwd_f32.hip', [], 'bvq_fakequant_bwd_f32.o'),
            ('bvq_weight_list.hip', [], 'bvq_weight_list.o')]
-HEADERS = ['bvq_common.h', 'bvq_quant_math.h', 'bvq_ties.h', 'bvq_sums.h', 'bvq_fakequant.h', 'bvq_fakequant_bwd.h',
+HEADERS = ['bvq_common.h', 'bvq_stat_epilogue.h', 'bvq_quant_math.h', 'bvq_ties.h', 'bvq_sums.h', 'bvq_fakequant.h', 'bvq_fakequant_bwd.h',
            os.path.join(ROOT, 'include', 'bvq.h')]
 
 FLAGS = [
diff --git a/brevitas_amd/csrc/bvq_autograd.cpp b/brevitas_amd/csrc/bvq_autograd.cpp
--- a/brevitas_amd/csrc/bvq_autograd.cpp
+++ b/brevitas_amd/csrc/bvq_autograd.cpp
@@ -24,6 +24,8 @@
   X(bvq_fakequant_bwd_stats_onepass)         \
   X(bvq_absmax_onepass_supported)            \
   X(bvq_absmax_scale_onepass)                \
+  X(bvq_absmax_fakequant_cluster_supported)  \
+  X(bvq_absmax_fakequant_cluster)            \
   X(bvq_stats_workspace_bytes)               \
   X(bvq_stats_pre)                           \
   X(bvq_absmax_scale)                        \
@@ -245,9 +247,17 @@
     const bool has_running = running.numel() > 0, has_arrive = arrive.numel() > 0;
     void* run_ptr = has_running ? running.data_ptr() : nullptr;
     const int run_dt = has_running ? code_of(running.scalar_type()) : BVQ_F32;
-    const bool onepass = has_arrive &&
+    at::Tensor y = at::empty(x.sizes(), x.options().dtype(dtype_of(d.ct_dtype)));
+    const int64_t words = (!sharded && has_arrive) ? p_bvq_absmax_fakequant_cluster_supported(&d, x.data_ptr(), y.data_ptr()) : 0;
+    const bool cluster = words > 0 && words <= arrive.numel();
+    const bool onepass = !cluster && has_arrive &&
                          p_bvq_absmax_onepass_supported(d.x_dtype, x.data_ptr(), d.outer, ch, d.inner);
-    if (onepass) {
+    if (cluster) {
+      check(p_bvq_absmax_fakequant_cluster(&d, x.data_ptr(), p.min_val, p.has_min, p.thr_fwd, stat.data_ptr(),
+                                           scale.data_ptr(), run_dt, run_ptr, p.momentum, p.first_batch, y.data_ptr(),
+                                           reinterpret_cast<uint32_t*>(arrive.data_ptr()), arrive.numel(), 0, nullptr, st),
+            "bvq_absmax_fakequant_cluster");
+    } else if (onepass) {
       check(p_bvq_absmax_scale_onepass(d.pre_op, d.x_dtype, x.data_ptr(), d.outer, ch, d.inner,
                                        sharded ? BVQ_F32 : d.x_dtype, sharded ? stat32.data_ptr() : stat.data_ptr(),
                                        p.min_val, p.has_min, p.thr_fwd, p.scale_dtype,
@@ -289,9 +299,9 @@
                                           p.first_batch, st),
             "bvq_scale_from_stat_running");
     }
-    at::Tensor y = at::empty(x.sizes(), x.options().dtype(dtype_of(d.ct_dtype)));
-    check(p_bvq_fakequant_fwd(&d, x.data_ptr(), scale.data_ptr(), zp.data_ptr(), y.data_ptr(), nullptr, st),
-          "bvq_fakequant_fwd");
+    if (!cluster)
+      check(p_bvq_fakequant_fwd(&d, x.data_ptr(), scale.data_ptr(), zp.data_ptr(), y.data_ptr(), nullptr, st),
+            "bvq_fakequant_fwd");
     ctx->save_for_backward({x, scale, zp, stat, int_threshold, arrive});
     ctx->saved_data["desc"] = desc_ints(p);
     ctx->saved_data["qrange"] = std::vector<double>{d.qmin, d.qmax, p.thr_bwd, p.thr_raw};
diff --git a/brevitas_amd/csrc/bvq_fakequant_fwd.hip b/brevitas_amd/csrc/bvq_fakequant_fwd.hip
--- a/brevitas_amd/csrc/bvq_fakequant_fwd.hip
+++ b/brevitas_amd/csrc/bvq_fakequant_fwd.hip
@@ -1,5 +1,6 @@
 
 #include "bvq_fakequant.h"
+#include "bvq_stat_epilogue.h"
 
 namespace bvq {
 
@@ -330,42 +331,41 @@
   for (int j = 0; j < kFusedSlots; ++j) ok[j] = lane + kWave * j < nch;
 }
 
-template <typename T, int RM>
-__device__ __forceinline__ void fused_channel(const FusedArgs& a, int32_t c, int r, int sl, const bool (&ok)[kFusedSlots],
-                                              float qmin, float qmax, int wave, int lane, int nwaves,
-                                              uint32_t* sh_max, uint32_t& sh_stat) {
+template <typename T>
+__device__ __forceinline__ void fused_load(const FusedArgs& a, int32_t c, int r, int sl, const bool (&ok)[kFusedSlots],
+                                           int lane, vec_t<T, elem<T>::vec> (&xv)[kFusedSlots]) {
   constexpr int VEC = elem<T>::vec;
   const int64_t base = ((int64_t)r * a.channels + c) * a.inner + (int64_t)sl * kFusedSliceChunks * VEC;
   const T* __restrict__ xp = reinterpret_cast<const T*>(a.x) + base;
-  T* __restrict__ yp = reinterpret_cast<T*>(a.y) + base;
-  vec_t<T, VEC> xv[kFusedSlots];
 #pragma unroll
   for (int j = 0; j < kFusedSlots; ++j)
     xv[j] = load_vec<T, VEC, true>(ok[j] ? xp + (int64_t)(lane + kWave * j) * VEC : reinterpret_cast<const T*>(a.x));
+}
+
+template <typename T>
+__device__ __forceinline__ uint32_t fused_key(const FusedArgs& a, const vec_t<T, elem<T>::vec> (&xv)[kFusedSlots],
+                                              const bool (&ok)[kFusedSlots]) {
   uint32_t m = 0;
 #pragma unroll
   for (int j = 0; j < kFusedSlots; ++j) {
     if (ok[j]) {
 #pragma unroll
-      for (int k = 0; k < VEC; ++k) {
+      for (int k = 0; k < elem<T>::vec; ++k) {
         const uint32_t b = a.pre_relu ? pre_abs_bits<T, true>(xv[j].v[k]) : pre_abs_bits<T, false>(xv[j].v[k]);
         m = b > m ? b : m;
       }
     }
   }
-  m = wave_max_u32(m);
-  if (lane == 0) sh_max[wave] = m;
-  __syncthreads();
-  if (threadIdx.x == 0) {
-    uint32_t bm = 0;
-    for (int w = 0; w < nwaves; ++w) bm = sh_max[w] > bm ? sh_max[w] : bm;
-    sh_stat = bm;
-  }
-  __syncthreads();
-  float stat;
-  float s = scale_from_key<T>(sh_stat, a.use_min, a.min_val, a.int_threshold, a.scale_dtype, stat);
-  if (threadIdx.x == 0) store_stat_scale<T>(a.stat_out, a.scale_out, a.scale_dtype, c, stat, s);
-  if (a.scalar_cast && !a.scale_pc) s = rnd<T>(s);
+  return m;
+}
+
+template <typename T, int RM>
+__device__ __forceinline__ void fused_apply(const FusedArgs& a, int32_t c, int r, int sl,
+                                            const vec_t<T, elem<T>::vec> (&xv)[kFusedSlots], const bool (&ok)[kFusedSlots],
+                                            float s, float qmin, float qmax, int lane) {
+  constexpr int VEC = elem<T>::vec;
+  const int64_t base = ((int64_t)r * a.channels + c) * a.inner + (int64_t)sl * kFusedSliceChunks * VEC;
+  T* __restrict__ yp = reinterpret_cast<T*>(a.y) + base;
   const int mode = a.round_mode;
   if constexpr (elem<T>::id == BVQ_BF16) {
     if (bf16_scale_ok(s)) {
@@ -392,6 +392,28 @@
     fused_quantize<T, RM, true>(xv, ok, yp, lane, div, s, qmin, qmax, mode);
   else
     fused_quantize<T, RM, false>(xv, ok, yp, lane, div, s, qmin, qmax, mode);
+}
+
+template <typename T, int RM>
+__device__ __forceinline__ void fused_channel(const FusedArgs& a, int32_t c, int r, int sl, const bool (&ok)[kFusedSlots],
+                                              float qmin, float qmax, int wave, int lane, int nwaves,
+                                              uint32_t* sh_max, uint32_t& sh_stat) {
+  vec_t<T, elem<T>::vec> xv[kFusedSlots];
+  fused_load<T>(a, c, r, sl, ok, lane, xv);
+  const uint32_t m = wave_max_u32(fused_key<T>(a, xv, ok));
+  if (lane == 0) sh_max[wave] = m;
+  __syncthreads();
+  if (threadIdx.x == 0) {
+    uint32_t bm = 0;
+    for (int w = 0; w < nwaves; ++w) bm = sh_max[w] > bm ? sh_max[w] : bm;
+    sh_stat = bm;
+  }
+  __syncthreads();
+  float stat;
+  float s = scale_from_key<T>(sh_stat, a.use_min, a.min_val, a.int_threshold, a.scale_dtype, stat);
+  if (threadIdx.x == 0) store_stat_scale<T>(a.stat_out, a.scale_out, a.scale_dtype, c, stat, s);
+  if (a.scalar_cast && !a.scale_pc) s = rnd<T>(s);
+  fused_apply<T, RM>(a, c, r, sl, xv, ok, s, qmin, qmax, lane);
 }
 
 template <typename T, int RM>
@@ -435,6 +457,147 @@
       qmax = rnd<T>(la.a[p].qmax);
     }
     fused_channel<T, RM>(la.a[p], pair - la.start[p], r, sl, ok, qmin, qmax, wave, lane, nwaves, sh_max, sh_stat);
+  }
+}
+
+
+#ifndef BVQ_CLUSTER_WAVES
+#define BVQ_CLUSTER_WAVES 16
+#endif
+#ifndef BVQ_CLUSTER_WAVES_PER_CU
+#define BVQ_CLUSTER_WAVES_PER_CU 16
+#endif
+#ifndef BVQ_CLUSTER_PREFETCH
+#define BVQ_CLUSTER_PREFETCH 1
+#endif
+constexpr int kClusterWaves = BVQ_CLUSTER_WAVES;
+constexpr int kClusterWavesPerCu = BVQ_CLUSTER_WAVES_PER_CU;
+constexpr bool kClusterPrefetch = BVQ_CLUSTER_PREFETCH != 0;
+constexpr int kClusterMaxMembers = kWave;
+constexpr uint32_t kClusterTag = 0x80000000u;
+constexpr uint64_t kClusterBudgetTicks = 200000;
+static_assert(kClusterWaves >= 1 && kClusterWaves * kWave <= 1024, "BVQ_CLUSTER_WAVES");
+
+struct ClusterArgs {
+  FusedArgs f;
+  ScaleEpilogue ep;
+  void* stat_out;
+  int32_t in_dtype;
+  uint32_t* key;
+  uint32_t* dep;
+  uint32_t* fallbacks;
+  int32_t members, nclusters, force_fallback;
+};
+
+template <typename T, int RM>
+__global__ __launch_bounds__(kClusterWaves * kWave, kClusterWavesPerCu / 4) void cluster_absmax_fakequant_kernel(ClusterArgs ca) {
+  constexpr int VEC = elem<T>::vec;
+  __shared__ uint32_t sh_max[kClusterWaves];
+  __shared__ uint32_t sh_stat, sh_ok;
+  const FusedArgs& a = ca.f;
+  const int lane = threadIdx.x & 63;
+  const int wave = __builtin_amdgcn_readfirstlane((int)(threadIdx.x >> 6));
+  const int32_t members = ca.members;
+  const int32_t member = (int32_t)blockIdx.x % members, cluster = (int32_t)blockIdx.x / members;
+  int r, sl;
+  bool ok[kFusedSlots];
+  fused_slice(a, member * kClusterWaves + wave, lane, r, sl, ok);
+  const float qmin = rnd<T>(a.qmin), qmax = rnd<T>(a.qmax);
+  int32_t c = cluster;
+  if (c >= a.channels) return;
+  vec_t<T, VEC> xv[kFusedSlots];
+  fused_load<T>(a, c, r, sl, ok, lane, xv);
+  for (; c < a.channels; c += ca.nclusters) {
+    const uint32_t m = wave_max_u32(fused_key<T>(a, xv, ok));
+    if (lane == 0) sh_max[wave] = m;
+    __syncthreads();
+    uint32_t* const keys = ca.key + (int64_t)c * members;
+    if (wave == 0) {
+      uint32_t bm = 0;
+      for (int w = 0; w < kClusterWaves; ++w) bm = sh_max[w] > bm ? sh_max[w] : bm;
+      if (lane == 0) __hip_atomic_store(keys + member, bm | kClusterTag, __ATOMIC_RELAXED, __HIP_MEMORY_SCOPE_AGENT);
+    }
+    const int32_t cn = c + ca.nclusters;
+    vec_t<T, VEC> xn[kFusedSlots];
+    if (kClusterPrefetch && cn < a.channels) fused_load<T>(a, cn, r, sl, ok, lane, xn);
+    if (wave == 0) {
+      bool done = false;
+      uint32_t v = 0;
+      if (!ca.force_fallback) {
+        const uint64_t t0 = __builtin_amdgcn_s_memrealtime();
+        for (;;) {
+          v = lane < members ? __hip_atomic_load(keys + lane, __ATOMIC_RELAXED, __HIP_MEMORY_SCOPE_AGENT) : kClusterTag;
+          if (__all((v & kClusterTag) != 0)) {
+            done = true;
+            break;
+          }
+          if (__builtin_amdgcn_s_memrealtime() - t0 > kClusterBudgetTicks) break;
+          __builtin_amdgcn_s_sleep(2);
+        }
+      }
+      v = wave_max_u32(v) & ~kClusterTag;
+      if (lane == 0) {
+        sh_stat = v;
+        sh_ok = done ? 1u : 0u;
+      }
+    }
+    __syncthreads();
+    if (!sh_ok) {
+      uint32_t fm = 0;
+      for (int q = wave; q < a.slices; q += kClusterWaves) {
+        int fr, fsl;
+        bool fok[kFusedSlots];
+        fused_slice(a, q, lane, fr, fsl, fok);
+        const T* xp = reinterpret_cast<const T*>(a.x) + ((int64_t)fr * a.channels + c) * a.inner +
+                      (int64_t)fsl * kFusedSliceChunks * VEC;
+        for (int j = 0; j < kFusedSlots; ++j) {
+          if (!fok[j]) break;
+          const vec_t<T, VEC> u = load_vec<T, VEC, false>(xp + (int64_t)(lane + kWave * j) * VEC);
+#pragma unroll
+          for (int k = 0; k < VEC; ++k) {
+            const uint32_t b = a.pre_relu ? pre_abs_bits<T, true>(u.v[k]) : pre_abs_bits<T, false>(u.v[k]);
+            fm = b > fm ? b : fm;
+          }
+        }
+      }
+      fm = wave_max_u32(fm);
+      if (lane == 0) sh_max[wave] = fm;
+      __syncthreads();
+      if (threadIdx.x == 0) {
+        uint32_t bm = 0;
+        for (int w = 0; w < kClusterWaves; ++w) bm = sh_max[w] > bm ? sh_max[w] : bm;
+        sh_stat = bm;
+        if (ca.fallbacks) __hip_atomic_fetch_add(ca.fallbacks, 1u, __ATOMIC_RELAXED, __HIP_MEMORY_SCOPE_AGENT);
+      }
+      __syncthreads();
+    }
+    const uint32_t key = sh_stat;
+    uint32_t before = 0;
+    if (wave == 0) {
+      if (lane == 0) {
+        if (!sh_ok) asm volatile("s_waitcnt vmcnt(0)" ::: "memory");
+        before = __hip_atomic_fetch_add(ca.dep + c, 1u, __ATOMIC_RELAXED, __HIP_MEMORY_SCOPE_AGENT);
+      }
+    }
+    float stat;
+    const float s = scale_from_key<T>(key, a.use_min, a.min_val, a.int_threshold, a.scale_dtype, stat);
+    if (member == 0 && threadIdx.x == 0) absmax_epilogue(ca.stat_out, ca.in_dtype, ca.in_dtype, ca.ep, c, key);
+    fused_apply<T, RM>(a, c, r, sl, xv, ok, s, qmin, qmax, lane);
+    if (wave == 0) {
+      before = __builtin_amdgcn_readfirstlane(before);
+      if (before + 1 == (uint32_t)members) {
+        if (lane < members) __hip_atomic_store(keys + lane, 0u, __ATOMIC_RELAXED, __HIP_MEMORY_SCOPE_AGENT);
+        if (lane == 0) __hip_atomic_store(ca.dep + c, 0u, __ATOMIC_RELAXED, __HIP_MEMORY_SCOPE_AGENT);
+      }
+    }
+    if (cn < a.channels) {
+      if constexpr (kClusterPrefetch) {
+#pragma unroll
+        for (int j = 0; j < kFusedSlots; ++j) xv[j] = xn[j];
+      } else {
+        fused_load<T>(a, cn, r, sl, ok, lane, xv);
+      }
+    }
   }
 }
 
@@ -626,6 +789,100 @@
   return BVQ_ERR_UNSUPPORTED;
 }
 
+struct ClusterPlan {
+  FusedPlan p;
+  int32_t members, nclusters;
+  int64_t words;
+};
+
+static bool cluster_plan(const bvq_quant_desc* d, const void* x, const void* y, ClusterPlan& cp) {
+  if (!(d->scale_per_channel && d->channels > 1) || d->channels >= ((int64_t)1 << 31)) return false;
+  const FusedShape f = fused_shape(d, x, y);
+  if (!f.ok) return false;
+  const uintptr_t bytes = (uintptr_t)(f.outer * f.channels * f.inner * dtype_size(d->x_dtype));
+  const uintptr_t xa = reinterpret_cast<uintptr_t>(x), ya = reinterpret_cast<uintptr_t>(y);
+  if (xa < ya + bytes && ya < xa + bytes) return false;
+  const int64_t cpr = f.inner / f.vec;
+  const int64_t spr = (cpr + kFusedSliceChunks - 1) / kFusedSliceChunks;
+  const int64_t slices = f.outer * spr;
+  const int64_t members = (slices + kClusterWaves - 1) / kClusterWaves;
+  if (cpr > (1 << 30) || members > kClusterMaxMembers) return false;
+  cp.p.cpr = (int32_t)cpr;
+  cp.p.spr = (int32_t)spr;
+  cp.p.slices = (int32_t)slices;
+  cp.p.waves = kClusterWaves;
+  cp.members = (int32_t)members;
+  const int64_t resident = (int64_t)num_cus() * kClusterWavesPerCu / kClusterWaves;
+  int64_t nc = resident / members;
+  nc = nc < 1 ? 1 : (nc > f.channels ? f.channels : nc);
+  cp.nclusters = (int32_t)nc;
+  cp.p.nblocks = (int32_t)(nc * members);
+  cp.words = f.channels * (members + 1);
+  return true;
+}
+
+extern "C" int64_t bvq_absmax_fakequant_cluster_supported(const bvq_quant_desc* d, const void* x, const void* y) {
+  if (validate(d)) return 0;
+  ClusterPlan cp;
+  return cluster_plan(d, x, y, cp) ? cp.words : 0;
+}
+
+extern "C" int bvq_absmax_fakequant_cluster(const bvq_quant_desc* d, const void* x, double min_val, int use_min,
+                                            double int_threshold, void* stat_out, void* scale_out, int run_dtype,
+                                            void* running, double momentum, int first_batch, void* y, uint32_t* arrive,
+                                            int64_t arrive_words, int flags, uint32_t* fallbacks,
+                                            bvq_stream_t stream) {
+  int rc = validate(d);
+  if (rc) return rc;
+  if (!x || !y || !stat_out || !scale_out || !arrive) {
+    set_error("bvq_absmax_fakequant_cluster: null pointer");
+    return BVQ_ERR_INVALID;
+  }
+  auto bad_dtype = [](int dt) { return dt < BVQ_F32 || dt > BVQ_F16; };
+  if ((running && bad_dtype(run_dtype)) || bad_dtype(d->scale_dtype) || !(int_threshold == int_threshold) ||
+      (flags & ~BVQ_CLUSTER_FORCE_FALLBACK)) {
+    set_error("bvq_absmax_fakequant_cluster: bad argument");
+    return BVQ_ERR_INVALID;
+  }
+  ClusterPlan cp;
+  if (!cluster_plan(d, x, y, cp)) {
+    set_error("bvq_absmax_fakequant_cluster: shape / layout not covered (bvq_absmax_fakequant_cluster_supported)");
+    return BVQ_ERR_UNSUPPORTED;
+  }
+  if (arrive_words < cp.words) {
+    set_error("bvq_absmax_fakequant_cluster: arrival buffer of %lld words, %lld needed", (long long)arrive_words,
+              (long long)cp.words);
+    return BVQ_ERR_WORKSPACE;
+  }
+  ClusterArgs ca = {};
+  ca.f = fused_args(d, cp.p, x, y, stat_out, scale_out, min_val, use_min, int_threshold);
+  ca.ep.scale_out = scale_out;
+  ca.ep.scale_dtype = d->scale_dtype;
+  ca.ep.use_min = use_min;
+  ca.ep.min_val = ca.f.min_val;
+  ca.ep.int_threshold = ca.f.int_threshold;
+  if (running) {
+    ca.ep.running = running;
+    ca.ep.run_dtype = run_dtype;
+    ca.ep.first_batch = first_batch;
+    ca.ep.one_minus_m = (float)(1.0 - momentum);
+    ca.ep.momentum = (float)momentum;
+  }
+  ca.stat_out = stat_out;
+  ca.in_dtype = d->x_dtype;
+  ca.key = arrive;
+  ca.dep = arrive + (int64_t)ca.f.channels * cp.members;
+  ca.fallbacks = fallbacks;
+  ca.members = cp.members;
+  ca.nclusters = cp.nclusters;
+  ca.force_fallback = (flags & BVQ_CLUSTER_FORCE_FALLBACK) ? 1 : 0;
+  hipStream_t st = (hipStream_t)stream;
+  rc = with_cols_variant(d, false, [&](auto t, auto rm, auto) {
+    cluster_absmax_fakequant_kernel<typename decltype(t)::type, rm><<<dim3((unsigned)cp.p.nblocks), dim3(kClusterWaves * kWave), 0, st>>>(ca);
+  });
+  return rc ? rc : check_launch("bvq_absmax_fakequant_cluster");
+}
+
 namespace bvq {
 int fused_list_fwd(int n, const bvq_quant_desc* descs, const bvq_weight_item* items, hipStream_t st) {
   FusedListArgs la = {};
diff --git a/brevitas_amd/csrc/bvq_stat_epilogue.h b/brevitas_amd/csrc/bvq_stat_epilogue.h
--- /dev/null
+++ b/brevitas_amd/csrc/bvq_stat_epilogue.h
@@ -0,0 +1,53 @@
+#pragma once
+
+#include "bvq_common.h"
+
+namespace bvq {
+
+__device__ __forceinline__ void store_stat(void* out, int out_dtype, int64_t idx, float v) {
+  if (out_dtype == BVQ_F32)
+    reinterpret_cast<float*>(out)[idx] = v;
+  else if (out_dtype == BVQ_BF16)
+    reinterpret_cast<bf16_t*>(out)[idx] = (bf16_t)v;
+  else
+    reinterpret_cast<f16_t*>(out)[idx] = (f16_t)v;
+}
+
+struct ScaleEpilogue {
+  void* scale_out;
+  int32_t scale_dtype;
+  int32_t use_min;
+  float min_val;
+  float int_threshold;
+  void* running;
+  int32_t run_dtype, first_batch;
+  float momentum, one_minus_m;
+};
+
+__device__ __forceinline__ float running_update(float r, float o, int run_dtype, int stat_dtype, float one_minus_m,
+                                                float m, int first) {
+  auto round_to = [](float v, int dt) {
+    return dt == BVQ_F32 ? v : (dt == BVQ_BF16 ? rnd<bf16_t>(v) : rnd<f16_t>(v));
+  };
+  if (first) return round_to(r * o, run_dtype);
+  r = round_to(r * one_minus_m, run_dtype);
+  const float u = round_to(o * m, stat_dtype);
+  return round_to(r + u, run_dtype);
+}
+
+__device__ __forceinline__ void absmax_epilogue(void* stat_out, int stat_dtype, int in_dtype, const ScaleEpilogue& ep,
+                                                int32_t c, uint32_t bits) {
+  const float v = in_dtype == BVQ_F16 ? (float)__builtin_bit_cast(f16_t, (uint16_t)bits) : __builtin_bit_cast(float, bits);
+  store_stat(stat_out, stat_dtype, c, v);
+  if (ep.scale_out) {
+    const float thr = (ep.use_min && v < ep.min_val) ? ep.min_val : v;
+    store_stat(ep.scale_out, ep.scale_dtype, c, thr / ep.int_threshold);
+  }
+  if (ep.running) {
+    const float run = load_scalar_as_f(ep.running, ep.run_dtype, c);
+    store_stat(ep.running, ep.run_dtype, c,
+               running_update(run, v, ep.run_dtype, stat_dtype, ep.one_minus_m, ep.momentum, ep.first_batch));
+  }
+}
+
+}
diff --git a/brevitas_amd/csrc/bvq_stats.hip b/brevitas_amd/csrc/bvq_stats.hip
--- a/brevitas_amd/csrc/bvq_stats.hip
+++ b/brevitas_amd/csrc/bvq_stats.hip
@@ -4,6 +4,7 @@
 #include "bvq_common.h"
 #include "bvq_ties.h"
 #include "bvq_sums.h"
+#include "bvq_stat_epilogue.h"
 
 namespace bvq {
 
@@ -338,15 +339,6 @@
   }
 }
 
-__device__ __forceinline__ void store_stat(void* out, int out_dtype, int64_t idx, float v) {
-  if (out_dtype == BVQ_F32)
-    reinterpret_cast<float*>(out)[idx] = v;
-  else if (out_dtype == BVQ_BF16)
-    reinterpret_cast<bf16_t*>(out)[idx] = (bf16_t)v;
-  else
-    reinterpret_cast<f16_t*>(out)[idx] = (f16_t)v;
-}
-
 __device__ __forceinline__ uint32_t order_key(float f) {
   const uint32_t u = __builtin_bit_cast(uint32_t, f);
   return (u >> 31) ? ~u : (u | 0x80000000u);
@@ -430,28 +422,6 @@
     store_stat(out, out_dtype, c, bad ? qn : order_key_value(kx));
     store_stat(out, out_dtype, (int64_t)channels + c, bad ? qn : -order_key_value(kn));
   }
-}
-
-struct ScaleEpilogue {
-  void* scale_out;
-  int32_t scale_dtype;
-  int32_t use_min;
-  float min_val;
-  float int_threshold;
-  void* running;
-  int32_t run_dtype, first_batch;
-  float momentum, one_minus_m;
-};
-
-__device__ __forceinline__ float running_update(float r, float o, int run_dtype, int stat_dtype, float one_minus_m,
-                                                float m, int first) {
-  auto round_to = [](float v, int dt) {
-    return dt == BVQ_F32 ? v : (dt == BVQ_BF16 ? rnd<bf16_t>(v) : rnd<f16_t>(v));
-  };
-  if (first) return round_to(r * o, run_dtype);
-  r = round_to(r * one_minus_m, run_dtype);
-  const float u = round_to(o * m, stat_dtype);
-  return round_to(r + u, run_dtype);
 }
 
 constexpr int64_t kFinishSlice = 4096;
@@ -570,18 +540,7 @@
 }
 
 __device__ __forceinline__ void absmax_finish(const ArriveArgs& r, const ScaleEpilogue& ep, int32_t c, uint32_t bits) {
-  const float v = r.in_dtype == BVQ_F16 ? (float)__builtin_bit_cast(f16_t, (uint16_t)bits)
-                                         : __builtin_bit_cast(float, bits);
-  store_stat(r.stat_out, r.stat_dtype, c, v);
-  if (ep.scale_out) {
-    const float thr = (ep.use_min && v < ep.min_val) ? ep.min_val : v;
-    store_stat(ep.scale_out, ep.scale_dtype, c, thr / ep.int_threshold);
-  }
-  if (ep.running) {
-    const float run = load_scalar_as_f(ep.running, ep.run_dtype, c);
-    store_stat(ep.running, ep.run_dtype, c,
-               running_update(run, v, ep.run_dtype, r.stat_dtype, ep.one_minus_m, ep.momentum, ep.first_batch));
-  }
+  absmax_epilogue(r.stat_out, r.stat_dtype, r.in_dtype, ep, c, bits);
 }
 
 __device__ __forceinline__ void absmax_arrive(const ArriveArgs& r, const ScaleEpilogue& ep, int32_t c, uint32_t m,
diff --git a/include/bvq.h b/include/bvq.h
--- a/include/bvq.h
+++ b/include/bvq.h
@@ -212,6 +212,13 @@
 int bvq_stats_fakequant_fwd(const bvq_quant_desc* desc, const void* x, double min_val, int use_min,
                             double int_threshold, void* stat_out, void* scale_out, void* y, void* workspace,
                             int64_t workspace_bytes, bvq_stream_t stream);
+
+#define BVQ_CLUSTER_FORCE_FALLBACK 1
+int64_t bvq_absmax_fakequant_cluster_supported(const bvq_quant_desc* desc, const void* x, const void* y);
+int bvq_absmax_fakequant_cluster(const bvq_quant_desc* desc, const void* x, double min_val, int use_min,
+                                 double int_threshold, void* stat_out, void* scale_out, int run_dtype, void* running,
+                                 double momentum, int first_batch, void* y, uint32_t* arrive, int64_t arrive_words,
+                                 int flags, uint32_t* fallbacks, bvq_stream_t stream);
 
 int64_t bvq_fakequant_bwd_workspace_bytes(const bvq_quant_desc* desc);
 
```

Result: faster. 549.2, median of 6 (+6.6%).
